# spencerkent/vision-transform-codes

Measured on AMD Instinct MI355X. Metric: patches/sec through 200-iter FISTA + dict update, 1024-atom dict, higher is better.
Workload: dtype f16x3

## Files before the change

### vision-transform-codes_amd/analysis_transforms/fully_connected/ista_fista.py

```python
import ctypes

import torch

import vtc_hip


def run(images, dictionary, sparsity_weight, num_iters, variant='fista',
        initial_codes=None, early_stopping_epsilon=None,
        nonnegative_only=False, hard_threshold=False, precision=None,
        stepsize=None):
  assert variant in ['ista', 'fista']
  lib = vtc_hip.load_library()
  images = vtc_hip.require_device_tensor(images, 'images').contiguous()
  dictionary = vtc_hip.require_device_tensor(
      dictionary, 'dictionary').contiguous()
  b, n = images.shape
  s = dictionary.shape[0]
  assert dictionary.shape[1] == n
  vtc_hip.prepare_device(images.device)
  if initial_codes is not None:
    initial_codes = vtc_hip.require_device_tensor(
        initial_codes, 'initial_codes').contiguous()
    assert tuple(initial_codes.shape) == (b, s)
  images = vtc_hip.aligned16(images)
  dictionary = vtc_hip.aligned16(dictionary)
  initial_codes = vtc_hip.aligned16(initial_codes)
  if num_iters < 1:
    raise UnboundLocalError(
        "local variable 'codes' referenced before assignment")

  mode = vtc_hip.threshold_mode(nonnegative_only, hard_threshold)
  prec = _resolve_precision(precision, b, n, s, early_stopping_epsilon)
  lam = float(sparsity_weight)
  eps = -1.0 if early_stopping_epsilon is None else float(
      early_stopping_epsilon)
  ws_bytes = lib.vtc_fc_ista_fista_workspace_bytes(b, n, s, prec)
  ws = vtc_hip.workspace(ws_bytes, images.device)
  codes = torch.empty((b, s), dtype=torch.float32, device=images.device)
  iters_run = ctypes.c_int(0)
  common = (int(num_iters), vtc_hip.variant_code(variant), mode, eps, prec,
            vtc_hip.ptr(ws), ws.numel(), ctypes.byref(iters_run),
            vtc_hip.current_stream(images.device))
  if (stepsize is None and early_stopping_epsilon is None and
      vtc_hip.device_stepsize_available(n)):
    eta_dev = vtc_hip.stepsize_on_device(
        vtc_hip.gram(dictionary, transpose_a=True), dictionary)
    with vtc_hip.timed_call(images.device):
      status = lib.vtc_fc_ista_fista_dev(
          vtc_hip.ptr(images), vtc_hip.ptr(dictionary),
          vtc_hip.ptr(initial_codes), vtc_hip.ptr(codes), b, n, s,
          vtc_hip.ptr(eta_dev), lam, *common)
    vtc_hip.check(status, 'vtc_fc_ista_fista_dev')
  else:
    if stepsize is None:
      stepsize = vtc_hip.stepsize_from_gram(
          vtc_hip.gram(dictionary, transpose_a=True), dictionary)
    with vtc_hip.timed_call(images.device):
      status = lib.vtc_fc_ista_fista(
          vtc_hip.ptr(images), vtc_hip.ptr(dictionary),
          vtc_hip.ptr(initial_codes), vtc_hip.ptr(codes), b, n, s,
          float(stepsize), lam, *common)
    vtc_hip.check(status, 'vtc_fc_ista_fista')
  run.last_iters = iters_run.value
  return codes


def _resolve_precision(precision, b, n, s, early_stopping_epsilon):
  name = precision if precision is not None else (
      vtc_hip.get_default_precision())
  if name == 'auto':
    fused_ok = (early_stopping_epsilon is None and n == 256 and
                s in (256, 512, 1024) and fused_available())
    tiled_ok = (n % 4 == 0 and s % 4 == 0 and b * s * n >= 240000000 and
                fused_available())
    streamed_ok = (early_stopping_epsilon is None and n == 256 and
                   s > 1024 and s % 256 == 0 and fused_available())
    if fused_ok or streamed_ok:
      return vtc_hip.F16X3
    small_ok = (early_stopping_epsilon is None and n == 64 and
                s in (64, 128, 192))
    if small_ok:
      return vtc_hip.F32
    if early_stopping_epsilon is None and (
        (n == 144 and s in (288, 576)) or (n == 64 and s in (256, 512))):
      return vtc_hip.F32
    return vtc_hip.F16X3 if tiled_ok else vtc_hip.F32
  return vtc_hip.PRECISIONS[name]


def fused_available():
  lib = vtc_hip.load_library()
  return lib.vtc_fc_ista_fista_workspace_bytes(32, 256, 1024,
                                               vtc_hip.BF16X3) > 256
```

### vision-transform-codes_amd/csrc/dict_update.hip

```cpp
#include "common.h"
#include "gemm_f32.h"

namespace vtc {

__global__ void slab_reduce_kernel(const float* __restrict__ slabs, int slices,
                                   int64_t count, float* __restrict__ out) {
  const int64_t stride = (int64_t)gridDim.x * blockDim.x;
  for (int64_t i = (int64_t)blockIdx.x * blockDim.x + threadIdx.x; i < count;
       i += stride) {
    float a[8] = {0.f, 0.f, 0.f, 0.f, 0.f, 0.f, 0.f, 0.f};
    int z = 0;
    for (; z + 8 <= slices; z += 8) {
#pragma unroll
      for (int u = 0; u < 8; ++u)
        a[u] = add_rn(a[u], slabs[(int64_t)(z + u) * count + i]);
    }
    for (int u = 0; z < slices; ++z, ++u)
      a[u] = add_rn(a[u], slabs[(int64_t)z * count + i]);
    out[i] = add_rn(add_rn(add_rn(a[0], a[1]), add_rn(a[2], a[3])),
                    add_rn(add_rn(a[4], a[5]), add_rn(a[6], a[7])));
  }
}

__global__ void slab_reduce_minus_kernel(const float* __restrict__ slabs,
                                         int slices, int64_t count,
                                         const float* __restrict__ X,
                                         float* __restrict__ out,
                                         unsigned* max_out) {
  const int64_t stride = (int64_t)gridDim.x * blockDim.x;
  float mx = 0.f;
  for (int64_t i = (int64_t)blockIdx.x * blockDim.x + threadIdx.x; i < count;
       i += stride) {
    float acc = slabs[i];
    for (int z = 1; z < slices; ++z) acc += slabs[(int64_t)z * count + i];
    const float r = sub_rn(acc, X[i]);
    out[i] = r;
    mx = fmaxf(mx, fabsf(r));
  }
  if (max_out) cx_publish_max_wave(mx, max_out);
}

int launch_slab_reduce_minus(const float* slabs, int slices, int64_t count,
                             const float* X, float* out, hipStream_t st,
                             unsigned* max_out) {
  if (count <= 0) return VTC_OK;
  int64_t blocks = ceil_div(count, 256);
  if (blocks > 4096) blocks = 4096;
  hipLaunchKernelGGL(slab_reduce_minus_kernel, dim3((unsigned)blocks),
                     dim3(256), 0, st, slabs, slices, count, X, out, max_out);
  VTC_LAUNCH_CHECK();
  return VTC_OK;
}

int launch_slab_reduce(const float* slabs, int slices, int64_t count,
                       float* out, hipStream_t st) {
  if (count <= 0) return VTC_OK;
  int64_t blocks = ceil_div(count, 256);
  if (blocks > 2048) blocks = 2048;
  hipLaunchKernelGGL(slab_reduce_kernel, dim3((unsigned)blocks), dim3(256), 0,
                     st, slabs, slices, count, out);
  VTC_LAUNCH_CHECK();
  return VTC_OK;
}

static int gradient_slices(int64_t b, int64_t n, int64_t s) {
  const int64_t tiles = ceil_div(s, kGemmBM) * ceil_div(n, kGemmBN);
  int64_t want = ceil_div(1024, tiles);
  const int64_t cap = ceil_div(b, 64);
  if (want > cap) want = cap;
  if (want > 128) want = 128;
  if (want < 1) want = 1;
  return gemm_effective_slices(b, (int)want);
}

__device__ __forceinline__ void fc_apply_row(
    float* __restrict__ D, const float* __restrict__ G,
    const float* __restrict__ hess, const float* __restrict__ P,
    float alignment_penalty, float batch_f, float stepsize, float lowest,
    int normalize, int64_t row, int64_t n, int lane) {
  float* d = D + row * n;
  const float* g = G + row * n;
  const float* p = P ? P + row * n : nullptr;
  const float denom = hess ? add_rn(hess[row], lowest) : 1.f;
  float sumsq = 0.f;
  for (int64_t j = lane; j < n; j += 64) {
    float grad = g[j] / batch_f;
    if (p) grad = add_rn(grad, mul_rn(alignment_penalty, p[j]));
    float step = mul_rn(stepsize, grad);
    if (hess) step = step / denom;
    const float v = sub_rn(d[j], step);
    d[j] = v;
    sumsq = fmaf(v, v, sumsq);
  }
  if (!normalize) return;
  const float norm = sqrtf(wave_sum(sumsq));
  for (int64_t j = lane; j < n; j += 64) d[j] = d[j] / norm;
}

__global__ __launch_bounds__(256) void fc_apply_kernel(
    float* __restrict__ D, const float* __restrict__ G,
    const float* __restrict__ hess, const float* __restrict__ P,
    float alignment_penalty, float batch_f, float stepsize, float lowest,
    int normalize, int64_t s, int64_t n, int rows_per_block) {
  const int lane = threadIdx.x & 63;
  const int64_t first = (int64_t)blockIdx.x * rows_per_block;
  const int64_t last = first + rows_per_block < s ? first + rows_per_block : s;
  for (int64_t row = first + (threadIdx.x >> 6); row < last; row += 4)
    fc_apply_row(D, G, hess, P, alignment_penalty, batch_f, stepsize, lowest,
                 normalize, row, n, lane);
}
constexpr int kMaxGroup = 256;
constexpr size_t kMaxAlignmentLds = 160 * 1024;

__global__ __launch_bounds__(256) void alignment_slot_kernel(
    const float* __restrict__ D, const int32_t* __restrict__ index,
    const uint8_t* __restrict__ valid, float* __restrict__ slot_grad,
    int64_t n, int m, int normalized) {
  extern __shared__ __attribute__((aligned(16))) float lds[];
  float* rows = lds;
  float* cosines = lds + (size_t)m * n;
  float* norms = cosines + m * m;
  const int g = blockIdx.x;
  const int32_t* idx = index + (int64_t)g * m;
  const uint8_t* ok = valid + (int64_t)g * m;
  int members = 0;
  for (int j = 0; j < m; ++j) members += ok[j] ? 1 : 0;
  for (int64_t e = threadIdx.x; e < (int64_t)members * n; e += blockDim.x) {
    const int r = (int)(e / n);
    const int64_t c = e % n;
    rows[e] = D[(int64_t)idx[r] * n + c];
  }
  __syncthreads();
  const int lane = threadIdx.x & 63, wave = threadIdx.x >> 6;
  for (int pair = wave; pair < members * members; pair += 4) {
    const int i = pair / members, j = pair % members;
    float acc = 0.f;
    for (int64_t c = lane; c < n; c += 64)
      acc = fmaf(rows[(int64_t)i * n + c], rows[(int64_t)j * n + c], acc);
    acc = wave_sum(acc);
    if (lane == 0) cosines[i * m + j] = acc;
  }
  __syncthreads();
  if (!normalized) {
    if (threadIdx.x < members)
      norms[threadIdx.x] = sqrtf(cosines[threadIdx.x * m + threadIdx.x]);
    __syncthreads();
  }
  for (int64_t e = threadIdx.x; e < (int64_t)members * n; e += blockDim.x) {
    const int i = (int)(e / n);
    const int64_t c = e % n;
    const float di = rows[(int64_t)i * n + c];
    float acc = 0.f;
    for (int j = 0; j < members; ++j) {
      const float dj = rows[(int64_t)j * n + c];
      float cs, toward_other, toward_self;
      if (normalized) {
        cs = cosines[i * m + j];
        toward_other = dj;
        toward_self = mul_rn(cs, di);
      } else {
        const float outer = mul_rn(norms[i], norms[j]);
        cs = cosines[i * m + j] / outer;
        toward_other = dj / outer;
        toward_self = mul_rn(cs / mul_rn(norms[i], norms[i]), di);
      }
      acc = add_rn(acc, mul_rn(sign_of(cs), sub_rn(toward_other, toward_self)));
    }
    slot_grad[((int64_t)g * m + i) * n + c] = acc;
  }
}

__global__ void rows_by_atom_sum_kernel(const float* __restrict__ slot_rows,
                                        const int32_t* __restrict__ atom_ptr,
                                        const int32_t* __restrict__ atom_slots,
                                        float* __restrict__ out, int64_t s,
                                        int64_t n) {
  const int64_t a = blockIdx.x;
  if (a >= s) return;
  const int beg = atom_ptr[a], end = atom_ptr[a + 1];
  for (int64_t c = threadIdx.x; c < n; c += blockDim.x) {
    float acc = 0.f;
    for (int t = beg; t < end; ++t)
      acc = add_rn(acc, slot_rows[(int64_t)atom_slots[t] * n + c]);
    out[a * n + c] = acc;
  }
}

__global__ __launch_bounds__(256) void energy_rows_kernel(
    const float* __restrict__ codes, int64_t b, int64_t s, int rows_per_chunk,
    float* __restrict__ partial) {
  const int64_t chunk = blockIdx.y;
  const int64_t j = (int64_t)blockIdx.x * blockDim.x + threadIdx.x;
  if (j >= s) return;
  const int64_t r0 = chunk * rows_per_chunk;
  int64_t r1 = r0 + rows_per_chunk;
  if (r1 > b) r1 = b;
  float acc = 0.f;
  for (int64_t r = r0; r < r1; ++r) {
    const float v = codes[r * s + j];
    acc = fmaf(v, v, acc);
  }
  partial[chunk * s + j] = acc;
}

__global__ __launch_bounds__(256) void energy_maps_kernel(
    const float* __restrict__ codes, int64_t s, int64_t positions,
    float* __restrict__ partial) {
  __shared__ float red[4];
  const int64_t map = blockIdx.x;
  const float* p = codes + map * positions;
  float acc = 0.f;
  for (int64_t i = threadIdx.x; i < positions; i += blockDim.x) {
    const float v = p[i];
    acc = fmaf(v, v, acc);
  }
  acc = wave_sum(acc);
  if ((threadIdx.x & 63) == 0) red[threadIdx.x >> 6] = acc;
  __syncthreads();
  if (threadIdx.x == 0) partial[map] = (red[0] + red[1]) + (red[2] + red[3]);
}

__global__ void hessian_ema_kernel(float* __restrict__ h,
                                   const float* __restrict__ energy,
                                   float batch_f, int64_t s) {
  const int64_t j = (int64_t)blockIdx.x * blockDim.x + threadIdx.x;
  if (j >= s) return;
  const float mean = energy[j] / batch_f;
  h[j] = add_rn(mul_rn(h[j], 0.99f), mean / 100.f);
}

static int energy_chunk_rows(int64_t b) {
  int64_t rows = ceil_div(b, 512);
  if (rows < 32) rows = 32;
  return (int)rows;
}


struct FcGradLayout {
  float* E;
  float* slabs;
  FcGradLayout(Carver& ws, int64_t b, int64_t n, int64_t s) {
    E = ws.take<float>((size_t)b * n);
    slabs = ws.take<float>((size_t)gradient_slices(b, n, s) * s * n);
  }
};

struct SlotGradLayout {
  float* slot_grad;
  SlotGradLayout(Carver& ws, int64_t slots, int64_t n) {
    slot_grad = ws.take<float>((size_t)(slots > 0 ? slots : 1) * n);
  }
};

struct EnergyLayout {
  int64_t chunks;
  float* partial;
  EnergyLayout(Carver& ws, int64_t b, int64_t s, int64_t positions) {
    chunks = positions > 1 ? b : ceil_div(b, energy_chunk_rows(b));
    partial = ws.take<float>((size_t)chunks * s);
  }
};

struct IcaMomentLayout {
  float* S;
  float* slabs;
  IcaMomentLayout(Carver& ws, int64_t b, int64_t s) {
    S = ws.take<float>((size_t)b * s);
    slabs = ws.take<float>((size_t)gradient_slices(b, s, s) * s * s);
  }
};

struct IcaApplyLayout {
  float* T;
  float* U;
  IcaApplyLayout(Carver& ws, int64_t s, int64_t n) {
    T = ws.take<float>((size_t)s * s);
    U = ws.take<float>((size_t)s * n);
  }
};

}

using namespace vtc;

extern "C" int vtc_gram(const float* a, int64_t rows, int64_t cols,
                        int transpose_a, float* gram, void* stream) {
  VTC_REQUIRE(a && gram, "vtc_gram: null pointer");
  VTC_REQUIRE(rows > 0 && cols > 0, "vtc_gram: bad sizes");
  hipStream_t st = as_stream(stream);
  if (transpose_a) {
    EpiStore e{gram, cols};
    return launch_gemm_f32<false, false>(a, cols, a, cols, cols, cols, rows, 1,
                                         e, st);
  }
  EpiStore e{gram, rows};
  return launch_gemm_f32<true, true>(a, cols, a, cols, rows, rows, cols, 1, e,
                                     st);
}

extern "C" size_t vtc_fc_dict_gradient_workspace_bytes(int64_t b, int64_t n,
                                                       int64_t s) {
  if (b <= 0 || n <= 0 || s <= 0) return 256;
  return measured_bytes<FcGradLayout>(b, n, s);
}

extern "C" int vtc_fc_dict_gradient(const float* images,
                                    const float* dictionary,
                                    const float* codes, float* grad_sum,
                                    int64_t b, int64_t n, int64_t s,
                                    void* workspace, size_t workspace_bytes,
                                    void* stream) {
  VTC_REQUIRE(images && dictionary && codes && grad_sum,
              "vtc_fc_dict_gradient: null pointer");
  VTC_REQUIRE(b > 0 && n > 0 && s > 0, "vtc_fc_dict_gradient: bad sizes");
  if (!workspace ||
      workspace_bytes < vtc_fc_dict_gradient_workspace_bytes(b, n, s)) {
    set_error("vtc_fc_dict_gradient: workspace too small");
    return VTC_ERR_WORKSPACE;
  }
  hipStream_t st = as_stream(stream);
  Carver ws(workspace);
  const FcGradLayout L(ws, b, n, s);
  const int slices = gradient_slices(b, n, s);
  EpiMinus e1{L.E, images, n, n};
  int rc = launch_gemm_f32<true, false>(codes, s, dictionary, n, b, n, s, 1,
                                        e1, st);
  if (rc != VTC_OK) return rc;
  if (b <= 512 && gemm_prefers_small(s, n)) {
    EpiStore direct{grad_sum, n};
    return launch_gemm_f32<false, false>(codes, s, L.E, n, s, n, b, 1, direct,
                                         st);
  }
  EpiSlab e2{L.slabs, s * n, n};
  rc = launch_gemm_f32<false, false>(codes, s, L.E, n, s, n, b, slices, e2, st);
  if (rc != VTC_OK) return rc;
  return launch_slab_reduce(L.slabs, slices, s * n, grad_sum, st);
}

__global__ void sign_kernel(const float* __restrict__ x, float* __restrict__ y,
                            int64_t count) {
  const int64_t stride = (int64_t)gridDim.x * blockDim.x;
  for (int64_t i = (int64_t)blockIdx.x * blockDim.x + threadIdx.x; i < count;
       i += stride)
    y[i] = sign_of(x[i]);
}

__global__ void ica_center_kernel(const float* __restrict__ moment_sum,
                                  float* __restrict__ T, float batch_f,
                                  int64_t s) {
  const int64_t total = s * s;
  const int64_t stride = (int64_t)gridDim.x * blockDim.x;
  for (int64_t i = (int64_t)blockIdx.x * blockDim.x + threadIdx.x; i < total;
       i += stride) {
    const float eye = (i / s == i % s) ? 1.f : 0.f;
    T[i] = sub_rn(moment_sum[i] / batch_f, eye);
  }
}

__global__ void axpy_rn_kernel(float* __restrict__ D,
                               const float* __restrict__ U, float stepsize,
                               int64_t count) {
  const int64_t stride = (int64_t)gridDim.x * blockDim.x;
  for (int64_t i = (int64_t)blockIdx.x * blockDim.x + threadIdx.x; i < count;
       i += stride)
    D[i] = add_rn(D[i], mul_rn(stepsize, U[i]));
}

static unsigned stream_grid(int64_t total) {
  int64_t blocks = ceil_div(total, 256);
  if (blocks > 4096) blocks = 4096;
  if (blocks < 1) blocks = 1;
  return (unsigned)blocks;
}

extern "C" int vtc_fc_residual(const float* images, const float* dictionary,
                               const float* codes, float* residual, int64_t b,
                               int64_t n, int64_t s, void* stream) {
  VTC_REQUIRE((images && dictionary && codes && residual) || b == 0,
              "vtc_fc_residual: null pointer");
  VTC_REQUIRE(b >= 0 && n > 0 && s > 0, "vtc_fc_residual: bad sizes");
  if (b == 0) return VTC_OK;
  EpiMinus e{residual, images, n, n};
  return launch_gemm_f32<true, false>(codes, s, dictionary, n, b, n, s, 1, e,
                                      as_stream(stream));
}

extern "C" size_t vtc_subspace_alignment_gradient_workspace_bytes(
    int64_t slots, int64_t n) {
  return measured_bytes<SlotGradLayout>(slots, n);
}

extern "C" int vtc_subspace_alignment_gradient(
    const float* dictionary, const int32_t* index, const uint8_t* valid,
    const int32_t* atom_ptr, const int32_t* atom_slots, float* penalty_grad,
    int64_t s, int64_t n, int64_t groups, int64_t m, int dict_is_normalized,
    void* workspace, size_t workspace_bytes, void* stream) {
  VTC_REQUIRE(dictionary && index && valid && atom_ptr && atom_slots &&
                  penalty_grad, "vtc_subspace_alignment_gradient: null");
  VTC_REQUIRE(s > 0 && n > 0 && groups > 0 && m > 0,
              "vtc_subspace_alignment_gradient: bad sizes");
  const size_t lds_bytes = ((size_t)m * n + (size_t)m * m + m) * sizeof(float);
  if (m > kMaxGroup || lds_bytes > kMaxAlignmentLds) {
    set_error("vtc_subspace_alignment_gradient: group of %lld atoms x %lld "
              "pixels exceeds the LDS tile", (long long)m, (long long)n);
    return VTC_ERR_UNSUPPORTED;
  }
  if (!workspace || workspace_bytes <
      vtc_subspace_alignment_gradient_workspace_bytes(groups * m, n)) {
    set_error("vtc_subspace_alignment_gradient: workspace too small");
    return VTC_ERR_WORKSPACE;
  }
  hipStream_t st = as_stream(stream);
  Carver ws(workspace);
  float* slot_grad = SlotGradLayout(ws, groups * m, n).slot_grad;
  VTC_HIP_CHECK(hipMemsetAsync(slot_grad, 0,
                               (size_t)groups * m * n * sizeof(float), st));
  if (lds_bytes > 64 * 1024)
    VTC_HIP_CHECK(hipFuncSetAttribute(
        reinterpret_cast<const void*>(alignment_slot_kernel),
        hipFuncAttributeMaxDynamicSharedMemorySize, (int)lds_bytes));
  hipLaunchKernelGGL(alignment_slot_kernel, dim3((unsigned)groups), dim3(256),
                     lds_bytes, st, dictionary, index, valid, slot_grad, n,
                     (int)m, dict_is_normalized);
  VTC_LAUNCH_CHECK();
  hipLaunchKernelGGL(rows_by_atom_sum_kernel, dim3((unsigned)s), dim3(256), 0,
                     st, slot_grad, atom_ptr, atom_slots, penalty_grad, s, n);
  VTC_LAUNCH_CHECK();
  return VTC_OK;
}

extern "C" int vtc_fc_dict_apply(float* dictionary, const float* grad_sum,
                                 const float* hessian_diagonal,
                                 const float* penalty_grad,
                                 float alignment_penalty, int64_t global_batch,
                                 float stepsize, float lowest_code_val,
                                 int normalize, int64_t s, int64_t n,
                                 void* stream) {
  VTC_REQUIRE(dictionary && grad_sum, "vtc_fc_dict_apply: null pointer");
  VTC_REQUIRE(s > 0 && n > 0 && global_batch > 0,
              "vtc_fc_dict_apply: bad sizes");
  int64_t rows = 32;
  while (rows > 4 && ((rows / 2) * n * 4) % 128 == 0) rows /= 2;
  if (reinterpret_cast<uintptr_t>(dictionary) % 128 != 0) rows = s;
  hipLaunchKernelGGL(fc_apply_kernel, dim3((unsigned)ceil_div(s, rows)),
                     dim3(256), 0, as_stream(stream), dictionary, grad_sum,
                     hessian_diagonal, penalty_grad, alignment_penalty,
                     (float)global_batch, stepsize, lowest_code_val, normalize,
                     s, n, (int)rows);
  VTC_LAUNCH_CHECK();
  return VTC_OK;
}

extern "C" size_t vtc_code_energy_workspace_bytes(int64_t b, int64_t s,
                                                  int64_t positions) {
  if (b <= 0 || s <= 0) return 256;
  return measured_bytes<EnergyLayout>(b, s, positions);
}

extern "C" int vtc_code_energy(const float* codes, int64_t b, int64_t s,
                               int64_t positions, float* energy,
                               void* workspace, size_t workspace_bytes,
                               void* stream) {
  VTC_REQUIRE(codes && energy, "vtc_code_energy: null pointer");
  VTC_REQUIRE(b > 0 && s > 0 && positions > 0, "vtc_code_energy: bad sizes");
  if (!workspace ||
      workspace_bytes < vtc_code_energy_workspace_bytes(b, s, positions)) {
    set_error("vtc_code_energy: workspace too small");
    return VTC_ERR_WORKSPACE;
  }
  hipStream_t st = as_stream(stream);
  Carver ws(workspace);
  const EnergyLayout L(ws, b, s, positions);
  const int64_t chunks = L.chunks;
  if (positions == 1) {
    const int rows = energy_chunk_rows(b);
    hipLaunchKernelGGL(energy_rows_kernel,
                       dim3((unsigned)ceil_div(s, 256), (unsigned)chunks),
                       dim3(256), 0, st, codes, b, s, rows, L.partial);
  } else {
    hipLaunchKernelGGL(energy_maps_kernel, dim3((unsigned)(b * s)), dim3(256),
                       0, st, codes, s, positions, L.partial);
  }
  VTC_LAUNCH_CHECK();
  return launch_slab_reduce(L.partial, (int)chunks, s, energy, st);
}

extern "C" int vtc_hessian_ema(float* hessian_diagonal, const float* energy,
                               int64_t global_batch, int64_t s, void* stream) {
  VTC_REQUIRE(hessian_diagonal && energy, "vtc_hessian_ema: null pointer");
  VTC_REQUIRE(s > 0 && global_batch > 0, "vtc_hessian_ema: bad sizes");
  hipLaunchKernelGGL(hessian_ema_kernel, dim3((unsigned)ceil_div(s, 256)),
                     dim3(256), 0, as_stream(stream), hessian_diagonal, energy,
                     (float)global_batch, s);
  VTC_LAUNCH_CHECK();
  return VTC_OK;
}

extern "C" size_t vtc_ica_moment_workspace_bytes(int64_t b, int64_t s) {
  if (b <= 0 || s <= 0) return 256;
  return measured_bytes<IcaMomentLayout>(b, s);
}

extern "C" int vtc_ica_moment(const float* codes, float* moment_sum, int64_t b,
                              int64_t s, void* workspace,
                              size_t workspace_bytes, void* stream) {
  VTC_REQUIRE(codes && moment_sum, "vtc_ica_moment: null pointer");
  VTC_REQUIRE(b > 0 && s > 0, "vtc_ica_moment: bad sizes");
  if (!workspace || workspace_bytes < vtc_ica_moment_workspace_bytes(b, s)) {
    set_error("vtc_ica_moment: workspace too small");
    return VTC_ERR_WORKSPACE;
  }
  hipStream_t st = as_stream(stream);
  Carver ws(workspace);
  const IcaMomentLayout L(ws, b, s);
  const int slices = gradient_slices(b, s, s);
  hipLaunchKernelGGL(sign_kernel, dim3(stream_grid(b * s)), dim3(256), 0, st,
                     codes, L.S, b * s);
  VTC_LAUNCH_CHECK();
  EpiSlab e{L.slabs, s * s, s};
  int rc = launch_gemm_f32<false, false>(codes, s, L.S, s, s, s, b, slices, e,
                                         st);
  if (rc != VTC_OK) return rc;
  return launch_slab_reduce(L.slabs, slices, s * s, moment_sum, st);
}

extern "C" size_t vtc_ica_apply_workspace_bytes(int64_t s, int64_t n) {
  if (s <= 0 || n <= 0) return 256;
  return measured_bytes<IcaApplyLayout>(s, n);
}

extern "C" int vtc_ica_apply(float* dictionary, const float* moment_sum,
                             int64_t global_batch, int64_t s, int64_t n,
                             float stepsize, void* workspace,
                             size_t workspace_bytes, void* stream) {
  VTC_REQUIRE(dictionary && moment_sum, "vtc_ica_apply: null pointer");
  VTC_REQUIRE(global_batch > 0 && s > 0 && n > 0, "vtc_ica_apply: bad sizes");
  if (!workspace || workspace_bytes < vtc_ica_apply_workspace_bytes(s, n)) {
    set_error("vtc_ica_apply: workspace too small");
    return VTC_ERR_WORKSPACE;
  }
  hipStream_t st = as_stream(stream);
  Carver ws(workspace);
  const IcaApplyLayout L(ws, s, n);
  hipLaunchKernelGGL(ica_center_kernel, dim3(stream_grid(s * s)), dim3(256), 0,
                     st, moment_sum, L.T, (float)global_batch, s);
  VTC_LAUNCH_CHECK();
  EpiStore e{L.U, n};
  int rc = launch_gemm_f32<true, false>(L.T, s, dictionary, n, s, n, s, 1, e,
                                        st);
  if (rc != VTC_OK) return rc;
  hipLaunchKernelGGL(axpy_rn_kernel, dim3(stream_grid(s * n)), dim3(256), 0,
                     st, dictionary, L.U, stepsize, s * n);
  VTC_LAUNCH_CHECK();
  return VTC_OK;
}
```

### vision-transform-codes_amd/csrc/fc_fused.h

```cpp
#pragma once
#include "common.h"
#include <vector>

namespace vtc {

bool fused_shape_supported(int64_t b, int64_t n, int64_t s, int precision);
size_t fused_workspace_bytes(int64_t b, int64_t n, int64_t s, int precision);
int run_fused(const float* images, const float* dictionary,
              const float* initial_codes, float* codes, int64_t b, int64_t n,
              int64_t s, float eta, const float* eta_dev,
              float sparsity_weight, int num_iters, int variant,
              int threshold, int precision, void* workspace,
              size_t workspace_bytes, int* iters_run, hipStream_t st);
int fused_max_iters();
const float* fista_beta_table_on_this_device();

void fista_betas(int num_iters, std::vector<float>* out);

}
```

### vision-transform-codes_amd/csrc/fc_fused.hip

```cpp
#include "fc_fused.h"
#include "fused_common.h"

#include <stdlib.h>
#include <mutex>
#include <vector>

namespace vtc {

struct FusedParams {
  const float* images;
  const float* init;
  float* codes;
  const uint4* packA[2];
  const uint4* packT[2];
  const float* betas;
  int64_t b;
  int s;
  int num_iters;
  int fista;
  float eta, cutoff;
  const float* eta_dev;
  float lam;
  const float* dscale;
  unsigned long long* stamps;
};

constexpr int kYxRow = 272;
constexpr int kRxRow = 528;
constexpr int kYxPart = 32 * kYxRow;
constexpr int kRxPart = 32 * kRxRow;

template <int NPH, int NP>
struct FusedLds {
  static constexpr int CREG_WANT = (NP == 1) ? 1 : 3;
  static constexpr int CREG = CREG_WANT < NPH ? CREG_WANT : NPH;
  static constexpr int CL = NPH - CREG;
  static constexpr int cst_bytes = CL * 16384;
  static constexpr int yx_bytes = 2 * NP * kYxPart;
  static constexpr int rx_bytes = NP * kRxPart;
  static constexpr int stat_bytes = 2 * 4 * 32 * 4;
  static constexpr int total = cst_bytes + yx_bytes + rx_bytes + stat_bytes;
};

template <int NPH, int NP, int MODE, bool F16 = false, bool STAMP = false>
__global__ __launch_bounds__(256, 1) void fused_fista_kernel(FusedParams P) {
  static_assert(!F16 || NP == 2, "the f16 split exists as three products only");
  using L = FusedLds<NPH, NP>;
  constexpr int CREG = L::CREG;
  constexpr int CR = CREG > 0 ? CREG : 1;
  constexpr int RING = (NP == 1) ? 16 : 8;
  extern __shared__ __attribute__((aligned(16))) char smem[];
  char* Cst = smem;
  char* Yx = smem + L::cst_bytes;
  char* Rx = Yx + L::yx_bytes;
  float* Stat = reinterpret_cast<float*>(Rx + L::rx_bytes);

  const int tid = threadIdx.x;
  const int lane = tid & 63;
  const int w = __builtin_amdgcn_readfirstlane(tid >> 6);
  const int r = lane & 31, h = lane >> 5;
  const int64_t patch = (int64_t)blockIdx.x * kFP + r;
  const bool live = patch < P.b;
  const int s = P.s;

  const unsigned pack_bytes_total = (unsigned)s * kFN * 2u;
  const unsigned a_wave_off = (unsigned)w * (16u * 64u * 16u);
  const unsigned t_wave_off = (unsigned)(2 * w) * (8u * 64u * 16u);
  __amdgpu_buffer_rsrc_t rsA[NP], rsT[NP];
#pragma unroll
  for (int part = 0; part < NP; ++part) {
    rsA[part] = __builtin_amdgcn_make_buffer_rsrc(
        (void*)((const char*)P.packA[part] + a_wave_off), 0,
        (int)(pack_bytes_total - a_wave_off), 0x00020000);
    rsT[part] = __builtin_amdgcn_make_buffer_rsrc(
        (void*)((const char*)P.packT[part] + t_wave_off), 0,
        (int)(pack_bytes_total - t_wave_off), 0x00020000);
  }
  const unsigned frag_voff = (unsigned)lane * 16u;
#define VTC_LOAD_A(part, p, i) \
  buffer_load16(rsA[part], frag_voff, (unsigned)(((4 * (p)) * 16 + (i)) * 1024))
#define VTC_LOAD_T(part, p, nb, ks) \
  buffer_load16(rsT[part], frag_voff,  \
                (unsigned)((((p) * 8 + (nb)) * 8 + (ks)) * 1024))

  const int yx_rd = r * kYxRow + 16 * h;
  const int yx_wr = r * kYxRow + 64 * w + 8 * h;
  const int rx_rd = r * kRxRow + 16 * h;
  const int rx_wr = r * kRxRow + 128 * w + 8 * h;
  const int cst_ln = w * 4096 + lane * 16;

  f32x16 Y[NPH];
  f32x16 Cr[CR];
  f32x16 Xr[2];
  f32x16 Racc[2];
  uint4 ring[NP][RING];

#pragma unroll
  for (int nb = 0; nb < 2; ++nb) {
#pragma unroll
    for (int g = 0; g < 4; ++g) {
      float4 v = make_float4(0.f, 0.f, 0.f, 0.f);
      if (live)
        v = *reinterpret_cast<const float4*>(
            P.images + patch * kFN + 64 * w + 32 * nb + 8 * g + 4 * h);
      Xr[nb][4 * g + 0] = v.x;
      Xr[nb][4 * g + 1] = v.y;
      Xr[nb][4 * g + 2] = v.z;
      Xr[nb][4 * g + 3] = v.w;
    }
  }
  const bool warm = (P.init != nullptr);
#pragma unroll
  for (int p = 0; p < NPH; ++p) {
#pragma unroll
    for (int g = 0; g < 4; ++g) {
      float4 v = make_float4(0.f, 0.f, 0.f, 0.f);
      if (warm && live)
        v = *reinterpret_cast<const float4*>(
            P.init + patch * s + kPhaseAtoms * p + 32 * w + 8 * g + 4 * h);
      Y[p][4 * g + 0] = v.x;
      Y[p][4 * g + 1] = v.y;
      Y[p][4 * g + 2] = v.z;
      Y[p][4 * g + 3] = v.w;
    }
  }
  float sigma_y = 1.f, inv_sigma_y = 1.f;
  float sigma_d = 1.f, inv_sigma_d = 1.f;
  if (F16) {
    float sx = 0.f, sy = 0.f;
#pragma unroll
    for (int nb = 0; nb < 2; ++nb)
#pragma unroll
      for (int e = 0; e < 16; ++e) sx += Xr[nb][e] * Xr[nb][e];
    if (warm) {
#pragma unroll
      for (int p = 0; p < NPH; ++p)
#pragma unroll
        for (int e = 0; e < 16; ++e) sy += Y[p][e] * Y[p][e];
    }
    sx += __shfl_xor(sx, 32, 64);
    sy += __shfl_xor(sy, 32, 64);
    float* red = reinterpret_cast<float*>(Rx);
    if (h == 0) {
      red[w * 64 + r] = sx;
      red[w * 64 + 32 + r] = sy;
    }
    __syncthreads();
    float tx = 0.f, ty = 0.f;
#pragma unroll
    for (int v = 0; v < 4; ++v) {
      tx += red[v * 64 + r];
      ty += red[v * 64 + 32 + r];
    }
    __syncthreads();
    const float m2 = fmaxf(tx, ty);
    int e2 = 0;
    if (m2 > 0.f && m2 < __builtin_inff()) e2 = ilogbf(m2) >> 1;
    e2 = e2 < -60 ? -60 : (e2 > 60 ? 60 : e2);
    sigma_y = ldexpf(1.f, 8 - e2);
    inv_sigma_y = ldexpf(1.f, e2 - 8);
    sigma_d = P.dscale[0];
    inv_sigma_d = P.dscale[1];
    const float sx_scale = sigma_d * sigma_y;
#pragma unroll
    for (int nb = 0; nb < 2; ++nb)
#pragma unroll
      for (int e = 0; e < 16; ++e) Xr[nb][e] *= sx_scale;
#pragma unroll
    for (int p = 0; p < NPH; ++p)
#pragma unroll
      for (int e = 0; e < 16; ++e) Y[p][e] *= sigma_y;
  }
  float eta = P.eta, cutoff_l = P.cutoff;
  if (P.eta_dev) {
    eta = *P.eta_dev;
    cutoff_l = mul_rn(P.lam, eta);
  }
  if (F16) {
    eta = eta * (0.5f * inv_sigma_d);
    cutoff_l = cutoff_l * sigma_y;
  }
  const float r_scale = F16 ? 2.f * inv_sigma_d : 1.f;
  int xr_calls = 0;
#pragma unroll
  for (int p = 0; p < NPH; ++p) {
#pragma unroll
    for (int g = 0; g < 4; ++g) {
      if (p < CREG) {
#pragma unroll
        for (int q = 0; q < 4; ++q)
          Cr[p < CREG ? p : 0][4 * g + q] = Y[p][4 * g + q];
      } else {
        *reinterpret_cast<float4*>(Cst + cst_ln + (p - CREG) * 16384 +
                                   g * 1024) =
            make_float4(Y[p][4 * g + 0], Y[p][4 * g + 1], Y[p][4 * g + 2],
                        Y[p][4 * g + 3]);
      }
    }
  }
#pragma unroll
  for (int nb = 0; nb < 2; ++nb)
#pragma unroll
    for (int e = 0; e < 16; ++e) Racc[nb][e] = 0.f;

  auto publish_y = [&](const f32x16& y, int buf) {
#pragma unroll
    for (int g = 0; g < 4; ++g) {
      const float v4[4] = {y[4 * g], y[4 * g + 1], y[4 * g + 2], y[4 * g + 3]};
      uint2 hi, lo;
      split_packed<F16, 4, NP == 2>(v4, hi, lo);
      char* dst = Yx + buf * NP * kYxPart + yx_wr + 16 * g;
      *reinterpret_cast<uint2*>(dst) = hi;
      if (NP == 2) *reinterpret_cast<uint2*>(dst + kYxPart) = lo;
    }
  };

#define VTC_SEG_IS_T(sg) (((sg) >= 2 && ((sg) % 2) == 0) || (sg) == 2 * NPH - 1)
#define VTC_SEG_PHASE(sg)                                        \
  ((sg) == 0 ? 0                                                 \
             : (sg) == 2 * NPH - 1 ? NPH - 1                     \
                                   : ((sg) % 2 ? ((sg) + 1) / 2 : (sg) / 2 - 1))
#define VTC_LOAD_SEG(part, sg, i)                                          \
  (VTC_SEG_IS_T(sg) ? VTC_LOAD_T(part, VTC_SEG_PHASE(sg), (i) & 1, (i) >> 1) \
                    : VTC_LOAD_A(part, VTC_SEG_PHASE(sg), (i)))
#define VTC_REFILL(sg, i)                                                   \
  {                                                                         \
    const int j_ = (i) + RING;                                              \
    const int sg_ = (j_ < 16) ? (sg) : (((sg) + 1) % (2 * NPH));            \
    const int i_ = (j_ < 16) ? j_ : j_ - 16;                                \
    _Pragma("unroll") for (int part = 0; part < NP; ++part)                 \
        ring[part][(i) % RING] = VTC_LOAD_SEG(part, sg_, i_);               \
  }

  auto step3 = [&](int p, int buf, bool pipe, int sg, auto&& between) {
    uint4 yb_next[NP];
#pragma unroll
    for (int part = 0; part < NP; ++part)
      yb_next[part] = *reinterpret_cast<const uint4*>(
          Yx + (buf * NP + part) * kYxPart + yx_rd);
#pragma unroll
    for (int ks = 0; ks < 8; ++ks) {
      uint4 yb[NP];
#pragma unroll
      for (int part = 0; part < NP; ++part) {
        yb[part] = yb_next[part];
        if (ks + 1 < 8)
          yb_next[part] = *reinterpret_cast<const uint4*>(
              Yx + (buf * NP + part) * kYxPart + yx_rd + 32 * (ks + 1));
      }
#pragma unroll
      for (int nb = 0; nb < 2; ++nb) {
        const int i = 2 * ks + nb;
        uint4 a[NP];
#pragma unroll
        for (int part = 0; part < NP; ++part)
          a[part] = pipe ? ring[part][i % RING] : VTC_LOAD_T(part, p, nb, ks);
        Racc[nb] = mfma16<F16>(a[0], yb[0], Racc[nb]);
        if constexpr (NP == 2) {
          Racc[nb] = mfma16<F16>(a[0], yb[1], Racc[nb]);
          Racc[nb] = mfma16<F16>(a[1], yb[0], Racc[nb]);
        }
        between(i);
        if (pipe) VTC_REFILL(sg, i)
        __builtin_amdgcn_sched_barrier(0);
      }
    }
  };
  auto nothing = [](int) {};

  auto exchange_r = [&]() {
    float v[2][16];
#pragma unroll
    for (int nb = 0; nb < 2; ++nb)
#pragma unroll
      for (int e = 0; e < 16; ++e) {
        v[nb][e] = sub_rn(Racc[nb][e], Xr[nb][e]);
        if (F16) v[nb][e] *= r_scale;
      }
    if (F16) {
      float m = 0.f;
#pragma unroll
      for (int nb = 0; nb < 2; ++nb)
#pragma unroll
        for (int e = 0; e < 16; ++e) m = fmaxf(m, fabsf(v[nb][e]));
      m = fmaxf(m, __shfl_xor(m, 32, 64));
      float f = 1.f;
      if (xr_calls > 0) {
        const float* prev = Stat + ((xr_calls - 1) & 1) * 128;
        const float Mx = fmaxf(fmaxf(prev[r], prev[32 + r]),
                               fmaxf(prev[64 + r], prev[96 + r]));
        if (Mx > 2048.f && Mx < __builtin_inff())
          f = ldexpf(1.f, 9 - ilogbf(Mx));
      }
      if (h == 0) Stat[(xr_calls & 1) * 128 + w * 32 + r] = m * f;
      ++xr_calls;
      if (__any(f != 1.f)) {
#pragma unroll
        for (int p = 0; p < NPH; ++p)
#pragma unroll
          for (int e = 0; e < 16; ++e) Y[p][e] *= f;
#pragma unroll
        for (int p = 0; p < CR; ++p)
#pragma unroll
          for (int e = 0; e < 16; ++e) Cr[p][e] *= f;
#pragma unroll
        for (int pl = 0; pl < L::CL; ++pl)
#pragma unroll
          for (int g = 0; g < 4; ++g) {
            float4* c4 = reinterpret_cast<float4*>(Cst + cst_ln + pl * 16384 +
                                                   g * 1024);
            float4 c = *c4;
            c.x *= f; c.y *= f; c.z *= f; c.w *= f;
            *c4 = c;
          }
#pragma unroll
        for (int nb = 0; nb < 2; ++nb)
#pragma unroll
          for (int e = 0; e < 16; ++e) {
            Xr[nb][e] *= f;
            v[nb][e] *= f;
          }
        cutoff_l *= f;
        inv_sigma_y *= 1.f / f;
      }
    }
#pragma unroll
    for (int nb = 0; nb < 2; ++nb) {
#pragma unroll
      for (int g = 0; g < 4; ++g) {
        const float v4[4] = {v[nb][4 * g], v[nb][4 * g + 1], v[nb][4 * g + 2],
                             v[nb][4 * g + 3]};
        uint2 hi, lo;
        split_packed<F16, 4, NP == 2>(v4, hi, lo);
        char* dst = Rx + rx_wr + 64 * nb + 16 * g;
        *reinterpret_cast<uint2*>(dst) = hi;
        if (NP == 2) *reinterpret_cast<uint2*>(dst + kRxPart) = lo;
      }
    }
#pragma unroll
    for (int nb = 0; nb < 2; ++nb)
#pragma unroll
      for (int e = 0; e < 16; ++e) Racc[nb][e] = 0.f;
    __syncthreads();
  };

  if (warm) {
#pragma unroll
    for (int p = 0; p < NPH; ++p) {
      publish_y(Y[p], p & 1);
      __syncthreads();
      step3(p, p & 1, false, 0, nothing);
    }
  }
  exchange_r();

#pragma unroll
  for (int i = 0; i < RING; ++i)
#pragma unroll
    for (int part = 0; part < NP; ++part)
      ring[part][i] = VTC_LOAD_SEG(part, 0, i);

  const bool fista = P.fista != 0;
  unsigned long long acc_t[5] = {0, 0, 0, 0, 0};
  unsigned long long t0 = 0, t1 = 0;
#define VTC_STAMP(slot)                    \
  if (STAMP) {                             \
    t1 = stamp_now();                      \
    acc_t[slot] += t1 - t0;                \
    t0 = t1;                               \
  }
  if (STAMP) t0 = stamp_now();

  f32x16 Gb[2];
  float4 cold4;
  float cn4[4];

  auto epilogue_elem = [&](int p, int e, const f32x16& Gp, float beta) {
    const int g = e >> 2, k = e & 3;
    if (MODE == 7) {
      const float cn = Y[p][e] + Gp[e];
      Y[p][e] = cn;
      cn4[k] = cn;
      if (k == 3) {
        if (p < CREG) {
#pragma unroll
          for (int q = 0; q < 4; ++q) Cr[p < CREG ? p : 0][4 * g + q] = cn4[q];
        } else {
          *reinterpret_cast<float4*>(Cst + cst_ln + (p - CREG) * 16384 +
                                     g * 1024) =
              make_float4(cn4[0], cn4[1], cn4[2], cn4[3]);
        }
      }
      return;
    }
    if (k == 0) {
      if (p < CREG) {
        cold4 = make_float4(Cr[p < CREG ? p : 0][4 * g + 0],
                            Cr[p < CREG ? p : 0][4 * g + 1],
                            Cr[p < CREG ? p : 0][4 * g + 2],
                            Cr[p < CREG ? p : 0][4 * g + 3]);
      } else {
        cold4 = *reinterpret_cast<const float4*>(
            Cst + cst_ln + (p - CREG) * 16384 + g * 1024);
      }
    }
    const float co = (k == 0) ? cold4.x : (k == 1) ? cold4.y
                   : (k == 2) ? cold4.z : cold4.w;
    const float c = sub_rn(Y[p][e], mul_rn(eta, Gp[e]));
    const float cn = shrink_fast<MODE>(c, cutoff_l);
    Y[p][e] = fista ? add_rn(cn, mul_rn(beta, sub_rn(cn, co))) : cn;
    cn4[k] = cn;
    if (k == 3) {
      if (p < CREG) {
#pragma unroll
        for (int q = 0; q < 4; ++q) Cr[p < CREG ? p : 0][4 * g + q] = cn4[q];
      } else {
        *reinterpret_cast<float4*>(Cst + cst_ln + (p - CREG) * 16384 +
                                   g * 1024) =
            make_float4(cn4[0], cn4[1], cn4[2], cn4[3]);
      }
      const float v4[4] = {Y[p][4 * g], Y[p][4 * g + 1], Y[p][4 * g + 2],
                           Y[p][4 * g + 3]};
      uint2 hi, lo;
      split_packed<F16, 4, NP == 2>(v4, hi, lo);
      char* dst = Yx + (p & 1) * NP * kYxPart + yx_wr + 16 * g;
      *reinterpret_cast<uint2*>(dst) = hi;
      if (NP == 2) *reinterpret_cast<uint2*>(dst + kYxPart) = lo;
    }
  };

  auto step1 = [&](int p, int sg, bool overlap, float beta) {
    f32x16& G = Gb[p & 1];
#pragma unroll
    for (int e = 0; e < 16; ++e) G[e] = 0.f;
    uint4 rb_next[NP];
#pragma unroll
    for (int part = 0; part < NP; ++part)
      rb_next[part] =
          *reinterpret_cast<const uint4*>(Rx + part * kRxPart + rx_rd);
#pragma unroll
    for (int i = 0; i < 16; ++i) {
      uint4 rb[NP];
#pragma unroll
      for (int part = 0; part < NP; ++part) {
        rb[part] = rb_next[part];
        if (i + 1 < 16)
          rb_next[part] = *reinterpret_cast<const uint4*>(
              Rx + part * kRxPart + rx_rd + 32 * (i + 1));
      }
      G = mfma16<F16>(ring[0][i % RING], rb[0], G);
      if constexpr (NP == 2) {
        G = mfma16<F16>(ring[0][i % RING], rb[1], G);
        G = mfma16<F16>(ring[1][i % RING], rb[0], G);
      }
      if (overlap) {
        epilogue_elem(p - 1, i, Gb[(p - 1) & 1], beta);
        __builtin_amdgcn_sched_barrier(0);
      }
      VTC_REFILL(sg, i)
      __builtin_amdgcn_sched_barrier(0);
    }
  };

  for (int it = 0; it < P.num_iters; ++it) {
    const float beta = fista ? P.betas[it] : 0.f;
    step1(0, 0, false, beta);
    VTC_STAMP(0)
#pragma unroll
    for (int p = 0; p < NPH; ++p) {
      if (p + 1 < NPH) {
        step1(p + 1, 2 * p + 1, true, beta);
        VTC_STAMP(0)
      }
      __syncthreads();
      VTC_STAMP(2)
      if (p + 2 == NPH) {
        step3(p, p & 1, true, 2 * p + 2, [&](int i) {
          epilogue_elem(NPH - 1, i, Gb[(NPH - 1) & 1], beta);
          __builtin_amdgcn_sched_barrier(0);
        });
      } else {
        step3(p, p & 1, true, (p + 1 < NPH) ? 2 * p + 2 : 2 * NPH - 1, nothing);
      }
      VTC_STAMP(3)
    }
    exchange_r();
    VTC_STAMP(4)
  }
  if (STAMP && lane == 0) {
#pragma unroll
    for (int k = 0; k < 5; ++k) atomicAdd(P.stamps + k, acc_t[k]);
    atomicAdd(P.stamps + 7, 1ull);
  }
#undef VTC_STAMP

#pragma unroll
  for (int p = 0; p < NPH; ++p) {
#pragma unroll
    for (int g = 0; g < 4; ++g) {
      float4 v;
      if (p < CREG) {
        v = make_float4(Cr[p < CREG ? p : 0][4 * g + 0],
                        Cr[p < CREG ? p : 0][4 * g + 1],
                        Cr[p < CREG ? p : 0][4 * g + 2],
                        Cr[p < CREG ? p : 0][4 * g + 3]);
      } else {
        v = *reinterpret_cast<const float4*>(Cst + cst_ln +
                                             (p - CREG) * 16384 + g * 1024);
      }
      if (F16) {
        v.x *= inv_sigma_y;
        v.y *= inv_sigma_y;
        v.z *= inv_sigma_y;
        v.w *= inv_sigma_y;
      }
      if (live)
        *reinterpret_cast<float4*>(P.codes + patch * s + kPhaseAtoms * p +
                                   32 * w + 8 * g + 4 * h) = v;
    }
  }
#undef VTC_LOAD_A
#undef VTC_LOAD_T
#undef VTC_LOAD_SEG
#undef VTC_REFILL
#undef VTC_SEG_IS_T
#undef VTC_SEG_PHASE
}

template <int NPH, int NP, int MODE, bool F16 = false, bool STAMP = false>
__global__ __launch_bounds__(256, 1) void fused_fista_kernel16(FusedParams P) {
  static_assert(!F16 || NP == 2, "the f16 split exists as three products only");
  using L = FusedLds<NPH, NP>;
  constexpr int CREG = L::CREG;
  constexpr int CR = CREG > 0 ? CREG : 1;
  constexpr int RING = (NP == 1) ? 16 : 8;
  constexpr int NPROD = (NP == 2) ? 3 : 1;
  extern __shared__ __attribute__((aligned(16))) char smem[];
  char* Cst = smem;
  char* Yx = smem + L::cst_bytes;
  char* Rx = Yx + L::yx_bytes;
  float* Stat = reinterpret_cast<float*>(Rx + L::rx_bytes);

  const int tid = threadIdx.x;
  const int lane = tid & 63;
  const int w = __builtin_amdgcn_readfirstlane(tid >> 6);
  const int c = lane & 15, q = lane >> 4;
  int64_t patch[2];
  bool live[2];
#pragma unroll
  for (int n = 0; n < 2; ++n) {
    patch[n] = (int64_t)blockIdx.x * kFP + 16 * n + c;
    live[n] = patch[n] < P.b;
  }
  const int s = P.s;

  const unsigned pack_bytes_total = (unsigned)s * kFN * 2u;
  const unsigned a_wave_off = (unsigned)w * (16u * 64u * 16u);
  const unsigned t_wave_off = (unsigned)(4 * w) * (4u * 64u * 16u);
  __amdgpu_buffer_rsrc_t rsA[NP], rsT[NP];
#pragma unroll
  for (int part = 0; part < NP; ++part) {
    rsA[part] = __builtin_amdgcn_make_buffer_rsrc(
        (void*)((const char*)P.packA[part] + a_wave_off), 0,
        (int)(pack_bytes_total - a_wave_off), 0x00020000);
    rsT[part] = __builtin_amdgcn_make_buffer_rsrc(
        (void*)((const char*)P.packT[part] + t_wave_off), 0,
        (int)(pack_bytes_total - t_wave_off), 0x00020000);
  }
  const unsigned frag_voff = (unsigned)lane * 16u;
#define VTC_LOAD_A(part, p, i) \
  buffer_load16(rsA[part], frag_voff, (unsigned)(((4 * (p)) * 16 + (i)) * 1024))
#define VTC_LOAD_T(part, p, nb, ks) \
  buffer_load16(rsT[part], frag_voff,  \
                (unsigned)((((p) * 16 + (nb)) * 4 + (ks)) * 1024))

  const int swap = ((c >> 2) ^ (c >> 3)) & 1;
  const int rd_chunk = 32 * (q >> 1) + 16 * ((q & 1) ^ swap);
  const int wr_chunk = 16 * ((q >> 1) ^ swap) + 8 * (q & 1);
  const int yx_rd = c * kYxRow + rd_chunk;
  const int yx_wr = c * kYxRow + 64 * w + wr_chunk;
  const int rx_rd = c * kRxRow + rd_chunk;
  const int rx_wr = c * kRxRow + 128 * w + wr_chunk;
  const int cst_ln = w * 4096 + lane * 16;
  constexpr int kYxHalf = 16 * kYxRow, kRxHalf = 16 * kRxRow;

  f32x16 Y[NPH];
  f32x16 Cr[CR];
  f32x4 Xr[4][2];
  f32x4 Racc[4][2];
  uint4 ring[NP][RING];

#pragma unroll
  for (int nb = 0; nb < 4; ++nb) {
#pragma unroll
    for (int n = 0; n < 2; ++n) {
      float4 v = make_float4(0.f, 0.f, 0.f, 0.f);
      if (live[n])
        v = *reinterpret_cast<const float4*>(P.images + patch[n] * kFN + 64 * w +
                                             16 * nb + 4 * q);
      Xr[nb][n][0] = v.x;
      Xr[nb][n][1] = v.y;
      Xr[nb][n][2] = v.z;
      Xr[nb][n][3] = v.w;
    }
  }
  const bool warm = (P.init != nullptr);
#pragma unroll
  for (int p = 0; p < NPH; ++p) {
#pragma unroll
    for (int g = 0; g < 4; ++g) {
      float4 v = make_float4(0.f, 0.f, 0.f, 0.f);
      if (warm && live[g & 1])
        v = *reinterpret_cast<const float4*>(P.init + patch[g & 1] * s +
                                             kPhaseAtoms * p + 32 * w +
                                             16 * (g >> 1) + 4 * q);
      Y[p][4 * g + 0] = v.x;
      Y[p][4 * g + 1] = v.y;
      Y[p][4 * g + 2] = v.z;
      Y[p][4 * g + 3] = v.w;
    }
  }
  float sigma_y[2] = {1.f, 1.f}, inv_sigma_y[2] = {1.f, 1.f};
  float sigma_d = 1.f, inv_sigma_d = 1.f;
  if (F16) {
    float sx[2] = {0.f, 0.f}, sy[2] = {0.f, 0.f};
#pragma unroll
    for (int nb = 0; nb < 4; ++nb)
#pragma unroll
      for (int n = 0; n < 2; ++n)
#pragma unroll
        for (int k = 0; k < 4; ++k) sx[n] += Xr[nb][n][k] * Xr[nb][n][k];
    if (warm) {
#pragma unroll
      for (int p = 0; p < NPH; ++p)
#pragma unroll
        for (int e = 0; e < 16; ++e) sy[(e >> 2) & 1] += Y[p][e] * Y[p][e];
    }
    float* red = reinterpret_cast<float*>(Rx);
#pragma unroll
    for (int n = 0; n < 2; ++n) {
      sx[n] += __shfl_xor(sx[n], 16, 64);
      sx[n] += __shfl_xor(sx[n], 32, 64);
      sy[n] += __shfl_xor(sy[n], 16, 64);
      sy[n] += __shfl_xor(sy[n], 32, 64);
      if (q == 0) {
        red[w * 64 + 16 * n + c] = sx[n];
        red[w * 64 + 32 + 16 * n + c] = sy[n];
      }
    }
    __syncthreads();
    float m2[2];
#pragma unroll
    for (int n = 0; n < 2; ++n) {
      float tx = 0.f, ty = 0.f;
#pragma unroll
      for (int v = 0; v < 4; ++v) {
        tx += red[v * 64 + 16 * n + c];
        ty += red[v * 64 + 32 + 16 * n + c];
      }
      m2[n] = fmaxf(tx, ty);
    }
    __syncthreads();
    sigma_d = P.dscale[0];
    inv_sigma_d = P.dscale[1];
#pragma unroll
    for (int n = 0; n < 2; ++n) {
      int e2 = 0;
      if (m2[n] > 0.f && m2[n] < __builtin_inff()) e2 = ilogbf(m2[n]) >> 1;
      e2 = e2 < -60 ? -60 : (e2 > 60 ? 60 : e2);
      sigma_y[n] = ldexpf(1.f, 8 - e2);
      inv_sigma_y[n] = ldexpf(1.f, e2 - 8);
      const float sx_scale = sigma_d * sigma_y[n];
#pragma unroll
      for (int nb = 0; nb < 4; ++nb)
#pragma unroll
        for (int k = 0; k < 4; ++k) Xr[nb][n][k] *= sx_scale;
    }
#pragma unroll
    for (int p = 0; p < NPH; ++p)
#pragma unroll
      for (int e = 0; e < 16; ++e) Y[p][e] *= sigma_y[(e >> 2) & 1];
  }
  float eta = P.eta, cutoff = P.cutoff;
  if (P.eta_dev) {
    eta = *P.eta_dev;
    cutoff = mul_rn(P.lam, eta);
  }
  float cutoff_l[2] = {cutoff, cutoff};
  if (F16) {
    eta = eta * (0.5f * inv_sigma_d);
    cutoff_l[0] = cutoff * sigma_y[0];
    cutoff_l[1] = cutoff * sigma_y[1];
  }
  const float r_scale = F16 ? 2.f * inv_sigma_d : 1.f;
  int xr_calls = 0;
#pragma unroll
  for (int p = 0; p < NPH; ++p) {
#pragma unroll
    for (int g = 0; g < 4; ++g) {
      if (p < CREG) {
#pragma unroll
        for (int k = 0; k < 4; ++k)
          Cr[p < CREG ? p : 0][4 * g + k] = Y[p][4 * g + k];
      } else {
        *reinterpret_cast<float4*>(Cst + cst_ln + (p - CREG) * 16384 +
                                   g * 1024) =
            make_float4(Y[p][4 * g + 0], Y[p][4 * g + 1], Y[p][4 * g + 2],
                        Y[p][4 * g + 3]);
      }
    }
  }
#pragma unroll
  for (int nb = 0; nb < 4; ++nb)
#pragma unroll
    for (int n = 0; n < 2; ++n)
#pragma unroll
      for (int k = 0; k < 4; ++k) Racc[nb][n][k] = 0.f;

  auto publish_group = [&](const f32x16& y, int g, int buf) {
    const float v4[4] = {y[4 * g], y[4 * g + 1], y[4 * g + 2], y[4 * g + 3]};
    uint2 hi, lo;
    split_packed<F16, 4, NP == 2>(v4, hi, lo);
    char* dst = Yx + buf * NP * kYxPart + yx_wr + 32 * (g >> 1) +
                kYxHalf * (g & 1);
    *reinterpret_cast<uint2*>(dst) = hi;
    if (NP == 2) *reinterpret_cast<uint2*>(dst + kYxPart) = lo;
  };

#define VTC_SEG_IS_T(sg) (((sg) >= 2 && ((sg) % 2) == 0) || (sg) == 2 * NPH - 1)
#define VTC_SEG_PHASE(sg)                                        \
  ((sg) == 0 ? 0                                                 \
             : (sg) == 2 * NPH - 1 ? NPH - 1                     \
                                   : ((sg) % 2 ? ((sg) + 1) / 2 : (sg) / 2 - 1))
#define VTC_LOAD_SEG(part, sg, i)                                          \
  (VTC_SEG_IS_T(sg) ? VTC_LOAD_T(part, VTC_SEG_PHASE(sg), (i) & 3, (i) >> 2) \
                    : VTC_LOAD_A(part, VTC_SEG_PHASE(sg), (i)))
#define VTC_REFILL(sg, i)                                                   \
  {                                                                         \
    const int j_ = (i) + RING;                                              \
    const int sg_ = (j_ < 16) ? (sg) : (((sg) + 1) % (2 * NPH));            \
    const int i_ = (j_ < 16) ? j_ : j_ - 16;                                \
    _Pragma("unroll") for (int part = 0; part < NP; ++part)                 \
        ring[part][(i) % RING] = VTC_LOAD_SEG(part, sg_, i_);               \
  }
#define VTC_MFMA_PAIR(acc0, acc1, a, b)                                     \
  _Pragma("unroll") for (int prod = 0; prod < NPROD; ++prod) {              \
    acc0 = mfma_k32<F16>(a[prod == 2], b[0][prod == 1], acc0);              \
    acc1 = mfma_k32<F16>(a[prod == 2], b[1][prod == 1], acc1);              \
  }

  auto step3 = [&](int p, int buf, bool pipe, int sg, auto&& between) {
    uint4 yb[2][NP], yb_next[2][NP];
#pragma unroll
    for (int n = 0; n < 2; ++n)
#pragma unroll
      for (int part = 0; part < NP; ++part)
        yb_next[n][part] = *reinterpret_cast<const uint4*>(
            Yx + (buf * NP + part) * kYxPart + yx_rd + kYxHalf * n);
#pragma unroll
    for (int i = 0; i < 16; ++i) {
      const int ks = i >> 2, nb = i & 3;
      if (nb == 0) {
#pragma unroll
        for (int n = 0; n < 2; ++n)
#pragma unroll
          for (int part = 0; part < NP; ++part) yb[n][part] = yb_next[n][part];
      }
      if (nb < 2 && ks + 1 < 4) {
#pragma unroll
        for (int part = 0; part < NP; ++part)
          yb_next[nb][part] = *reinterpret_cast<const uint4*>(
              Yx + (buf * NP + part) * kYxPart + yx_rd + kYxHalf * nb +
              64 * (ks + 1));
      }
      uint4 a[NP];
#pragma unroll
      for (int part = 0; part < NP; ++part)
        a[part] = pipe ? ring[part][i % RING] : VTC_LOAD_T(part, p, nb, ks);
      VTC_MFMA_PAIR(Racc[nb][0], Racc[nb][1], a, yb)
      between(i);
      if (pipe) VTC_REFILL(sg, i)
      __builtin_amdgcn_sched_barrier(0);
    }
  };
  auto nothing = [](int) {};

  auto exchange_r = [&]() {
    float v[4][2][4];
#pragma unroll
    for (int nb = 0; nb < 4; ++nb)
#pragma unroll
      for (int n = 0; n < 2; ++n)
#pragma unroll
        for (int k = 0; k < 4; ++k) {
          v[nb][n][k] = sub_rn(Racc[nb][n][k], Xr[nb][n][k]);
          if (F16) v[nb][n][k] *= r_scale;
        }
    if (F16) {
      float f[2] = {1.f, 1.f};
#pragma unroll
      for (int n = 0; n < 2; ++n) {
        float m = 0.f;
#pragma unroll
        for (int nb = 0; nb < 4; ++nb)
#pragma unroll
          for (int k = 0; k < 4; ++k) m = fmaxf(m, fabsf(v[nb][n][k]));
        m = fmaxf(m, __shfl_xor(m, 16, 64));
        m = fmaxf(m, __shfl_xor(m, 32, 64));
        const int row = 16 * n + c;
        if (xr_calls > 0) {
          const float* prev = Stat + ((xr_calls - 1) & 1) * 128;
          const float Mx = fmaxf(fmaxf(prev[row], prev[32 + row]),
                                 fmaxf(prev[64 + row], prev[96 + row]));
          if (Mx > 2048.f && Mx < __builtin_inff())
            f[n] = ldexpf(1.f, 9 - ilogbf(Mx));
        }
        if (q == 0) Stat[(xr_calls & 1) * 128 + w * 32 + row] = m * f[n];
      }
      ++xr_calls;
      if (__any(f[0] != 1.f || f[1] != 1.f)) {
#pragma unroll
        for (int p = 0; p < NPH; ++p)
#pragma unroll
          for (int e = 0; e < 16; ++e) Y[p][e] *= f[(e >> 2) & 1];
#pragma unroll
        for (int p = 0; p < CR; ++p)
#pragma unroll
          for (int e = 0; e < 16; ++e) Cr[p][e] *= f[(e >> 2) & 1];
#pragma unroll
        for (int pl = 0; pl < L::CL; ++pl)
#pragma unroll
          for (int g = 0; g < 4; ++g) {
            float4* c4 = reinterpret_cast<float4*>(Cst + cst_ln + pl * 16384 +
                                                   g * 1024);
            float4 cc = *c4;
            const float fg = f[g & 1];
            cc.x *= fg; cc.y *= fg; cc.z *= fg; cc.w *= fg;
            *c4 = cc;
          }
#pragma unroll
        for (int n = 0; n < 2; ++n) {
#pragma unroll
          for (int nb = 0; nb < 4; ++nb)
#pragma unroll
            for (int k = 0; k < 4; ++k) {
              Xr[nb][n][k] *= f[n];
              v[nb][n][k] *= f[n];
            }
          cutoff_l[n] *= f[n];
          inv_sigma_y[n] *= 1.f / f[n];
        }
      }
    }
#pragma unroll
    for (int nb = 0; nb < 4; ++nb) {
#pragma unroll
      for (int n = 0; n < 2; ++n) {
        const float v4[4] = {v[nb][n][0], v[nb][n][1], v[nb][n][2], v[nb][n][3]};
        uint2 hi, lo;
        split_packed<F16, 4, NP == 2>(v4, hi, lo);
        char* dst = Rx + rx_wr + 32 * nb + kRxHalf * n;
        *reinterpret_cast<uint2*>(dst) = hi;
        if (NP == 2) *reinterpret_cast<uint2*>(dst + kRxPart) = lo;
      }
    }
#pragma unroll
    for (int nb = 0; nb < 4; ++nb)
#pragma unroll
      for (int n = 0; n < 2; ++n)
#pragma unroll
        for (int k = 0; k < 4; ++k) Racc[nb][n][k] = 0.f;
    __syncthreads();
  };

  if (warm) {
#pragma unroll
    for (int p = 0; p < NPH; ++p) {
#pragma unroll
      for (int g = 0; g < 4; ++g) publish_group(Y[p], g, p & 1);
      __syncthreads();
      step3(p, p & 1, false, 0, nothing);
    }
  }
  exchange_r();

#pragma unroll
  for (int i = 0; i < RING; ++i)
#pragma unroll
    for (int part = 0; part < NP; ++part)
      ring[part][i] = VTC_LOAD_SEG(part, 0, i);

  const bool fista = P.fista != 0;
  unsigned long long acc_t[5] = {0, 0, 0, 0, 0};
  unsigned long long t0 = 0, t1 = 0;
#define VTC_STAMP(slot)                    \
  if (STAMP) {                             \
    t1 = stamp_now();                      \
    acc_t[slot] += t1 - t0;                \
    t0 = t1;                               \
  }
  if (STAMP) t0 = stamp_now();

  f32x4 Gb[2][4];
  float4 cold4;
  float cn4[4];

  auto epilogue_elem = [&](int p, int e, const f32x4 (&Gp)[4], float beta) {
    const int g = e >> 2, k = e & 3;
    if (MODE == 7) {
      const float cn = Y[p][e] + Gp[g][k];
      Y[p][e] = cn;
      cn4[k] = cn;
      if (k == 3) {
        if (p < CREG) {
#pragma unroll
          for (int j = 0; j < 4; ++j) Cr[p < CREG ? p : 0][4 * g + j] = cn4[j];
        } else {
          *reinterpret_cast<float4*>(Cst + cst_ln + (p - CREG) * 16384 +
                                     g * 1024) =
              make_float4(cn4[0], cn4[1], cn4[2], cn4[3]);
        }
      }
      return;
    }
    if (k == 0) {
      if (p < CREG) {
        cold4 = make_float4(Cr[p < CREG ? p : 0][4 * g + 0],
                            Cr[p < CREG ? p : 0][4 * g + 1],
                            Cr[p < CREG ? p : 0][4 * g + 2],
                            Cr[p < CREG ? p : 0][4 * g + 3]);
      } else {
        cold4 = *reinterpret_cast<const float4*>(
            Cst + cst_ln + (p - CREG) * 16384 + g * 1024);
      }
    }
    const float co = (k == 0) ? cold4.x : (k == 1) ? cold4.y
                   : (k == 2) ? cold4.z : cold4.w;
    const float cv = sub_rn(Y[p][e], mul_rn(eta, Gp[g][k]));
    const float cn = shrink_fast<MODE>(cv, cutoff_l[g & 1]);
    Y[p][e] = fista ? add_rn(cn, mul_rn(beta, sub_rn(cn, co))) : cn;
    cn4[k] = cn;
    if (k == 3) {
      if (p < CREG) {
#pragma unroll
        for (int j = 0; j < 4; ++j) Cr[p < CREG ? p : 0][4 * g + j] = cn4[j];
      } else {
        *reinterpret_cast<float4*>(Cst + cst_ln + (p - CREG) * 16384 +
                                   g * 1024) =
            make_float4(cn4[0], cn4[1], cn4[2], cn4[3]);
      }
      publish_group(Y[p], g, p & 1);
    }
  };

  auto step1 = [&](int p, int sg, bool overlap, float beta) {
    f32x4 (&G)[4] = Gb[p & 1];
#pragma unroll
    for (int g = 0; g < 4; ++g)
#pragma unroll
      for (int k = 0; k < 4; ++k) G[g][k] = 0.f;
    uint4 rb[2][NP], rb_next[2][NP];
#pragma unroll
    for (int n = 0; n < 2; ++n)
#pragma unroll
      for (int part = 0; part < NP; ++part)
        rb_next[n][part] = *reinterpret_cast<const uint4*>(
            Rx + part * kRxPart + rx_rd + kRxHalf * n);
#pragma unroll
    for (int i = 0; i < 16; ++i) {
      const int ks = i >> 1, m = i & 1;
      if (m == 0) {
#pragma unroll
        for (int n = 0; n < 2; ++n)
#pragma unroll
          for (int part = 0; part < NP; ++part) rb[n][part] = rb_next[n][part];
      }
      if (ks + 1 < 8) {
#pragma unroll
        for (int part = 0; part < NP; ++part)
          rb_next[m][part] = *reinterpret_cast<const uint4*>(
              Rx + part * kRxPart + rx_rd + kRxHalf * m + 64 * (ks + 1));
      }
      uint4 a[NP];
#pragma unroll
      for (int part = 0; part < NP; ++part) a[part] = ring[part][i % RING];
      VTC_MFMA_PAIR(G[2 * m], G[2 * m + 1], a, rb)
      if (overlap) {
        epilogue_elem(p - 1, i, Gb[(p - 1) & 1], beta);
        __builtin_amdgcn_sched_barrier(0);
      }
      VTC_REFILL(sg, i)
      __builtin_amdgcn_sched_barrier(0);
    }
  };

  for (int it = 0; it < P.num_iters; ++it) {
    const float beta = fista ? P.betas[it] : 0.f;
    step1(0, 0, false, beta);
    VTC_STAMP(0)
#pragma unroll
    for (int p = 0; p < NPH; ++p) {
      if (p + 1 < NPH) {
        step1(p + 1, 2 * p + 1, true, beta);
        VTC_STAMP(0)
      }
      __syncthreads();
      VTC_STAMP(2)
      if (p + 2 == NPH) {
        step3(p, p & 1, true, 2 * p + 2, [&](int i) {
          epilogue_elem(NPH - 1, i, Gb[(NPH - 1) & 1], beta);
          __builtin_amdgcn_sched_barrier(0);
        });
      } else {
        step3(p, p & 1, true, (p + 1 < NPH) ? 2 * p + 2 : 2 * NPH - 1, nothing);
      }
      VTC_STAMP(3)
    }
    exchange_r();
    VTC_STAMP(4)
  }
  if (STAMP && lane == 0) {
#pragma unroll
    for (int k = 0; k < 5; ++k) atomicAdd(P.stamps + k, acc_t[k]);
    atomicAdd(P.stamps + 7, 1ull);
  }
#undef VTC_STAMP

#pragma unroll
  for (int p = 0; p < NPH; ++p) {
#pragma unroll
    for (int g = 0; g < 4; ++g) {
      float4 v;
      if (p < CREG) {
        v = make_float4(Cr[p < CREG ? p : 0][4 * g + 0],
                        Cr[p < CREG ? p : 0][4 * g + 1],
                        Cr[p < CREG ? p : 0][4 * g + 2],
                        Cr[p < CREG ? p : 0][4 * g + 3]);
      } else {
        v = *reinterpret_cast<const float4*>(Cst + cst_ln +
                                             (p - CREG) * 16384 + g * 1024);
      }
      if (F16) {
        v.x *= inv_sigma_y[g & 1];
        v.y *= inv_sigma_y[g & 1];
        v.z *= inv_sigma_y[g & 1];
        v.w *= inv_sigma_y[g & 1];
      }
      if (live[g & 1])
        *reinterpret_cast<float4*>(P.codes + patch[g & 1] * s + kPhaseAtoms * p +
                                   32 * w + 16 * (g >> 1) + 4 * q) = v;
    }
  }
#undef VTC_LOAD_A
#undef VTC_LOAD_T
#undef VTC_LOAD_SEG
#undef VTC_REFILL
#undef VTC_MFMA_PAIR
#undef VTC_SEG_IS_T
#undef VTC_SEG_PHASE
}

}

namespace vtc {

static int phases_for(int64_t s) { return (int)(s / kPhaseAtoms); }

bool fused_shape_supported(int64_t b, int64_t n, int64_t s, int precision) {
  if (n != kFN || b <= 0) return false;
  if (s % kPhaseAtoms != 0) return false;
  const int nph = phases_for(s);
  if (!(nph == 2 || nph == 4 || nph == 8)) return false;
  return precision == VTC_BF16 || precision == VTC_BF16X3 ||
         precision == VTC_F16X3;
}

static int fused_parts(int precision) { return precision == VTC_BF16 ? 1 : 2; }

struct FusedLayout {
  unsigned short* packs[4] = {nullptr, nullptr, nullptr, nullptr};
  float* dscale;
  FusedLayout(Carver& ws, int64_t s, int parts) {
    for (int part = 0; part < parts; ++part) {
      packs[2 * part] = ws.take<unsigned short>((size_t)s * kFN);
      packs[2 * part + 1] = ws.take<unsigned short>((size_t)s * kFN);
    }
    dscale = ws.take<float>(2);
  }
};

size_t fused_workspace_bytes(int64_t b, int64_t n, int64_t s, int precision) {
  if (!fused_shape_supported(b, n, s, precision)) return 256;
  return measured_bytes<FusedLayout>(s, fused_parts(precision));
}

static bool default_tile16(int precision) {
  return precision == VTC_F16X3 || precision == VTC_BF16;
}
static bool use_tile16(int precision) {
  const char* v = getenv("VTC_FUSED_TILE");
  if (v && v[0] == '1' && v[1] == '6' && v[2] == 0) return true;
  if (v && v[0] == '3' && v[1] == '2' && v[2] == 0) return false;
  return default_tile16(precision);
}

template <int NPH, int NP, int MODE, bool F16, bool STAMP, bool TILE16>
static auto fused_kernel() {
  if constexpr (TILE16)
    return fused_fista_kernel16<NPH, NP, MODE, F16, STAMP>;
  else
    return fused_fista_kernel<NPH, NP, MODE, F16, STAMP>;
}

template <int NPH, int NP, int MODE, bool F16, bool TILE16>
static int launch_fused(const FusedParams& P, hipStream_t st) {
  using L = FusedLds<NPH, NP>;
  auto kernel = fused_kernel<NPH, NP, MODE, F16, false, TILE16>();
  static unsigned long long configured = 0;
  if (first_use_on_this_device(&configured)) {
    VTC_HIP_CHECK(hipFuncSetAttribute(
        reinterpret_cast<const void*>(kernel),
        hipFuncAttributeMaxDynamicSharedMemorySize, L::total));
  }
  const unsigned grid = (unsigned)ceil_div(P.b, kFP);
  hipLaunchKernelGGL(kernel, dim3(grid), dim3(256), L::total, st, P);
  VTC_LAUNCH_CHECK();
  return VTC_OK;
}

template <int NPH, int NP, bool F16, bool TILE16>
static int launch_stamped(FusedParams P, hipStream_t st) {
  using L = FusedLds<NPH, NP>;
  static const bool no_epilogue = getenv("VTC_FUSED_NOEPI") != nullptr;
  auto kernel = no_epilogue
                    ? fused_kernel<NPH, NP, 7, F16, true, TILE16>()
                    : fused_kernel<NPH, NP, VTC_SOFT, F16, true, TILE16>();
  unsigned long long* dev = nullptr;
  VTC_HIP_CHECK(hipMalloc(&dev, 8 * sizeof(unsigned long long)));
  VTC_HIP_CHECK(hipMemsetAsync(dev, 0, 8 * sizeof(unsigned long long), st));
  VTC_HIP_CHECK(hipFuncSetAttribute(
      reinterpret_cast<const void*>(kernel),
      hipFuncAttributeMaxDynamicSharedMemorySize, L::total));
  P.stamps = dev;
  hipLaunchKernelGGL(kernel, dim3((unsigned)ceil_div(P.b, kFP)), dim3(256),
                     L::total, st, P);
  VTC_LAUNCH_CHECK();
  unsigned long long host[8];
  VTC_HIP_CHECK(hipMemcpyAsync(host, dev, sizeof(host), hipMemcpyDeviceToHost,
                               st));
  VTC_HIP_CHECK(hipStreamSynchronize(st));
  VTC_HIP_CHECK(hipFree(dev));
  const char* names[5] = {"step1+epi", "epi-alone", "barrier", "step3",
                          "exchange"};
  double total = 0;
  for (int k = 0; k < 5; ++k) total += (double)host[k];
  const double per = (double)host[7] * P.num_iters * NPH;
  for (int k = 0; k < 5; ++k)
    fprintf(stderr, "[vtc stamps] %-9s %5.1f%%  %8.0f cycles/phase/wave\n",
            names[k], 100.0 * host[k] / total, host[k] / per);
  return VTC_OK;
}

template <int NPH, int NP, bool F16, bool TILE16>
static int dispatch_mode(const FusedParams& P, int threshold, hipStream_t st) {
  static const bool stamps = getenv("VTC_FUSED_STAMPS") != nullptr;
  if (stamps && threshold == VTC_SOFT && NPH == 8 && NP == 2)
    return launch_stamped<NPH, NP, F16, TILE16>(P, st);
  switch (threshold) {
    case VTC_SOFT: return launch_fused<NPH, NP, VTC_SOFT, F16, TILE16>(P, st);
    case VTC_SOFT_NONNEG:
      return launch_fused<NPH, NP, VTC_SOFT_NONNEG, F16, TILE16>(P, st);
    case VTC_HARD: return launch_fused<NPH, NP, VTC_HARD, F16, TILE16>(P, st);
    default: return launch_fused<NPH, NP, VTC_HARD_NONNEG, F16, TILE16>(P, st);
  }
}

template <int NP, bool F16, bool TILE16>
static int dispatch_phases(const FusedParams& P, int threshold,
                           hipStream_t st) {
  switch (phases_for(P.s)) {
    case 2: return dispatch_mode<2, NP, F16, TILE16>(P, threshold, st);
    case 4: return dispatch_mode<4, NP, F16, TILE16>(P, threshold, st);
    case 8: return dispatch_mode<8, NP, F16, TILE16>(P, threshold, st);
  }
  set_error("fused FISTA: unsupported atom count %d", P.s);
  return VTC_ERR_UNSUPPORTED;
}

constexpr int kBetaTable = 16384;
const float* fista_beta_table_on_this_device() {
  static float* tables[64] = {nullptr};
  static std::mutex guard;
  int dev = 0;
  if (hipGetDevice(&dev) != hipSuccess || dev < 0 || dev > 63) return nullptr;
  std::lock_guard<std::mutex> lock(guard);
  if (tables[dev]) return tables[dev];
  std::vector<float> host;
  fista_betas(kBetaTable, &host);
  float* table = nullptr;
  if (hipMalloc(&table, sizeof(float) * kBetaTable) != hipSuccess)
    return nullptr;
  if (hipMemcpy(table, host.data(), sizeof(float) * kBetaTable,
                hipMemcpyHostToDevice) != hipSuccess) {
    (void)hipFree(table);
    return nullptr;
  }
  tables[dev] = table;
  return table;
}

int fused_max_iters() { return kBetaTable; }

int run_fused(const float* images, const float* dictionary,
              const float* initial_codes, float* codes, int64_t b, int64_t n,
              int64_t s, float eta, const float* eta_dev,
              float sparsity_weight, int num_iters, int variant,
              int threshold, int precision, void* workspace,
              size_t workspace_bytes, int* iters_run, hipStream_t st) {
  if (!fused_shape_supported(b, n, s, precision)) {
    set_error("fused FISTA: unsupported shape");
    return VTC_ERR_UNSUPPORTED;
  }
  if (num_iters > kBetaTable) {
    set_error("fused FISTA: at most %d iterations per call", kBetaTable);
    return VTC_ERR_UNSUPPORTED;
  }
  if (!workspace ||
      workspace_bytes < fused_workspace_bytes(b, n, s, precision)) {
    set_error("fused FISTA: workspace too small");
    return VTC_ERR_WORKSPACE;
  }
  const float* betas_dev = fista_beta_table_on_this_device();
  if (!betas_dev) {
    set_error("fused FISTA: could not place the momentum table on the device");
    return VTC_ERR_HIP;
  }
  const int parts = fused_parts(precision);
  const bool f16 = (precision == VTC_F16X3);
  Carver ws(workspace);
  FusedParams P;
  const FusedLayout L(ws, s, parts);
  unsigned short* const* packs = L.packs;
  float* dscale = L.dscale;
  if (f16) {
    hipLaunchKernelGGL(dictionary_scale_kernel, dim3(1), dim3(1024), 0, st,
                       dictionary, (int64_t)s * kFN, dscale);
    VTC_LAUNCH_CHECK();
  }
  const bool tile16 = use_tile16(precision);
  auto pack = f16 ? (tile16 ? pack_dictionary_kernel<true, true>
                            : pack_dictionary_kernel<true, false>)
                  : (tile16 ? pack_dictionary_kernel<false, true>
                            : pack_dictionary_kernel<false, false>);
  hipLaunchKernelGGL(pack, dim3(256), dim3(256), 0, st, dictionary, (int)s,
                     packs[0], packs[1], packs[2], packs[3], dscale);
  VTC_LAUNCH_CHECK();
  P.images = images;
  P.init = initial_codes;
  P.codes = codes;
  for (int part = 0; part < 2; ++part) {
    P.packA[part] = reinterpret_cast<const uint4*>(packs[2 * (part % parts)]);
    P.packT[part] =
        reinterpret_cast<const uint4*>(packs[2 * (part % parts) + 1]);
  }
  P.betas = betas_dev;
  P.b = b;
  P.s = (int)s;
  P.num_iters = num_iters;
  P.fista = (variant == VTC_FISTA) ? 1 : 0;
  P.eta = eta;
  P.eta_dev = eta_dev;
  P.lam = sparsity_weight;
  P.cutoff = sparsity_weight * eta;
  P.dscale = dscale;
  P.stamps = nullptr;
  int rc;
  if (tile16)
    rc = f16          ? dispatch_phases<2, true, true>(P, threshold, st)
         : parts == 2 ? dispatch_phases<2, false, true>(P, threshold, st)
                      : dispatch_phases<1, false, true>(P, threshold, st);
  else
    rc = f16          ? dispatch_phases<2, true, false>(P, threshold, st)
         : parts == 2 ? dispatch_phases<2, false, false>(P, threshold, st)
                      : dispatch_phases<1, false, false>(P, threshold, st);
  if (rc == VTC_OK && iters_run) *iters_run = num_iters;
  return rc;
}

}

extern "C" int vtc_init(void) {
  if (!vtc::fista_beta_table_on_this_device()) {
    vtc::set_error("vtc_init: could not place the momentum table on the device");
    return VTC_ERR_HIP;
  }
  return VTC_OK;
}
```

### vision-transform-codes_amd/csrc/fc_inference.hip

```cpp
#include "common.h"
#include "gemm_f32.h"
#include "gemm_x3.h"
#include "epi_prox.h"
#include "fc_fused.h"
#include "fused_stream.h"
#include "fc_small.h"

#include <math.h>
#include <vector>

namespace vtc {

struct EpiProx {
  float* Y;
  float* C;
  int64_t ld;
  float eta, cutoff, beta;
  int mode;
  int fista;
  double* delta_sum;
  double local;
  const float* eta_dev = nullptr;
  float lam = 0.f;
  float* Yo = nullptr;
  float* Co = nullptr;
  __device__ __forceinline__ void resolve() {
    if (eta_dev) {
      eta = *eta_dev;
      cutoff = mul_rn(lam, eta);
    }
  }

  static constexpr bool kElemFetch = true;
  struct Fetched {
    float y, c;
  };
  __device__ __forceinline__ Fetched fetch(int64_t row, int64_t col) const {
    const int64_t i = row * ld + col;
    Fetched f;
    f.y = Y[i];
    f.c = fista ? C[i] : 0.f;
    return f;
  }
  __device__ __forceinline__ void apply(int64_t row, int64_t col, float g, int,
                                        const Fetched& f) {
    const int64_t i = row * ld + col;
    const float c = shrink(sub_rn(f.y, mul_rn(eta, g)), cutoff, mode);
    float d;
    if (fista) {
      d = sub_rn(c, f.c);
      Yo[i] = add_rn(c, mul_rn(beta, d));
    } else {
      d = sub_rn(c, f.y);
    }
    Co[i] = c;
    if (delta_sum) local += (double)(fabsf(d) / eta);
  }
  __device__ __forceinline__ void block_end() {
    if (!delta_sum) return;
    const double w = wave_sum(local);
    if ((threadIdx.x & 63) == 0) atomicAdd(delta_sum, w);
  }
};

void fista_betas(int num_iters, std::vector<float>* out) {
  out->resize(num_iters);
  double t = 1.0;
  for (int k = 0; k < num_iters; ++k) {
    const double t_next = (1.0 + sqrt(1.0 + 4.0 * t * t)) / 2.0;
    (*out)[k] = (float)((t - 1.0) / t_next);
    t = t_next;
  }
}

int launch_transpose(const float* in, float* out, int64_t rows, int64_t cols,
                     hipStream_t st);

static size_t generic_workspace_bytes(int64_t b, int64_t n, int64_t s) {
  return measured_bytes<TiledIstaLayout>(b, n, s);
}

static int run_generic(const float* images, const float* dictionary,
                       const float* initial_codes, float* codes, int64_t b,
                       int64_t n, int64_t s, float eta, const float* eta_dev,
                       float lam, int num_iters, int variant, int threshold,
                       float eps, bool x3, bool f16, void* workspace,
                       size_t workspace_bytes, int* iters_run, hipStream_t st) {
  const float cutoff = lam * eta;
  if (workspace_bytes < generic_workspace_bytes(b, n, s) || !workspace) {
    set_error("vtc_fc_ista_fista: workspace too small (%zu < %zu)",
              workspace_bytes, generic_workspace_bytes(b, n, s));
    return VTC_ERR_WORKSPACE;
  }
  Carver ws(workspace);
  const TiledIstaLayout L(ws, b, n, s);
  float* R = L.R;
  float* Dt = L.Dt;
  if (x3 && (n % 4 != 0 || s % 4 != 0)) {
    set_error("vtc_fc_ista_fista: bf16x3 outside the fused kernel needs n "
              "and s to be multiples of 4");
    return VTC_ERR_UNSUPPORTED;
  }
  if (x3 && ((reinterpret_cast<uintptr_t>(dictionary) |
              reinterpret_cast<uintptr_t>(codes)) & 15) != 0)
    x3 = false;
  const int k1_slices = x3 ? gemm_x3_want_slices(b, n, s) : 1;
  double* delta_sum = L.delta_sum;
  unsigned* state = L.state;
  f16 = f16 && x3;
  float* dscale = f16 ? reinterpret_cast<float*>(state) : nullptr;
  unsigned* y_slot[2] = {state + 64, state + 64 + kCxMaxSlotWords};
  unsigned* r_slot[2] = {state + 64 + 2 * kCxMaxSlotWords,
                         state + 64 + 3 * kCxMaxSlotWords};
  if (f16) {
    VTC_HIP_CHECK(hipMemsetAsync(state, 0, kX3StateWords * sizeof(unsigned),
                                 st));
    hipLaunchKernelGGL(cx_array_scale_kernel, dim3(1), dim3(1024), 0, st,
                       dictionary, s * n, dscale);
    VTC_LAUNCH_CHECK();
    if (initial_codes) {
      hipLaunchKernelGGL(cx_array_max_kernel, dim3(1024), dim3(256), 0, st,
                         initial_codes, b * s, y_slot[0]);
      VTC_LAUNCH_CHECK();
    }
  }

  const bool fista = (variant == VTC_FISTA);
  float* Y = fista ? L.Y : codes;
  if (x3) {
    if (!gemm_x3_usable(Y, s, Dt, s) || !gemm_x3_usable(R, n, dictionary, n)) {
      set_error("vtc_fc_ista_fista: split tiles on an unaligned operand");
      return VTC_ERR_INVALID_ARGUMENT;
    }
    int rc = launch_transpose(dictionary, Dt, s, n, st);
    if (rc != VTC_OK) return rc;
  }
  const size_t code_bytes = (size_t)b * s * sizeof(float);
  if (initial_codes) {
    VTC_HIP_CHECK(hipMemcpyAsync(codes, initial_codes, code_bytes,
                                 hipMemcpyDeviceToDevice, st));
    if (fista)
      VTC_HIP_CHECK(hipMemcpyAsync(Y, initial_codes, code_bytes,
                                   hipMemcpyDeviceToDevice, st));
  } else {
    VTC_HIP_CHECK(hipMemsetAsync(codes, 0, code_bytes, st));
    if (fista) VTC_HIP_CHECK(hipMemsetAsync(Y, 0, code_bytes, st));
  }

  std::vector<float> betas;
  fista_betas(num_iters, &betas);
  int done = 0;
  float* Cin = codes;
  float* Cout = L.Cout;
  float* Yout = L.Yout;
  for (int k = 0; k < num_iters; ++k) {
    if (!fista) Y = Cin;
    EpiMinus e1{R, images, n, n};
    X3Scale sc1, sc2;
    if (f16) {
      sc1.b_scale = sc2.b_scale = dscale;
      sc1.a_max = y_slot[k & 1];
      sc1.clear = y_slot[(k + 1) & 1];
      sc2.a_max = r_slot[k & 1];
      sc2.clear = r_slot[(k + 1) & 1];
    }
    int rc;
    if (x3 && k1_slices > 1) {
      EpiSlab es{L.slabs, b * n, n};
      rc = launch_gemm_x3(Y, s, Dt, s, b, n, s, es, st, k1_slices, sc1);
      if (rc == VTC_OK)
        rc = launch_slab_reduce_minus(L.slabs, k1_slices, b * n, images, R, st,
                                      f16 ? r_slot[k & 1] : nullptr);
    } else if (x3 && f16) {
      EpiMinusMax e1m{R, images, n, n, r_slot[k & 1]};
      rc = launch_gemm_x3(Y, s, Dt, s, b, n, s, e1m, st, 1, sc1);
    } else if (x3) {
      rc = launch_gemm_x3(Y, s, Dt, s, b, n, s, e1, st, 1, sc1);
    } else {
      rc = launch_gemm_f32<true, false>(Y, s, dictionary, n, b, n, s, 1, e1,
                                        st);
    }
    if (rc != VTC_OK) return rc;
    if (eps >= 0.f)
      VTC_HIP_CHECK(hipMemsetAsync(delta_sum, 0, sizeof(double), st));
    const bool wide_ok = s % 4 == 0 &&
                         (reinterpret_cast<uintptr_t>(Y) & 15) == 0 &&
                         (reinterpret_cast<uintptr_t>(codes) & 15) == 0;
    if (x3 || (wide_ok && !gemm_prefers_small(b, s))) {
      EpiGroupProx<1, true> e2{Y, Cin, s, eta, cutoff,
                               fista ? betas[k] : 0.f, fista ? 1 : 0,
                               eps >= 0.f ? delta_sum : nullptr, 0.0,
                               threshold, eta_dev, lam};
      e2.Yo = fista ? Yout : Cout;
      e2.Co = Cout;
      if (f16) {
        EpiGroupProx<1, true, true> e2t{Y, Cin, s, eta, cutoff,
                                        fista ? betas[k] : 0.f, fista ? 1 : 0,
                                        eps >= 0.f ? delta_sum : nullptr, 0.0,
                                        threshold, eta_dev, lam};
        e2t.Yo = e2.Yo;
        e2t.Co = e2.Co;
        e2t.track.max_out = y_slot[(k + 1) & 1];
        rc = launch_gemm_x3(R, n, dictionary, n, b, s, n, e2t, st, 1, sc2);
      } else {
        rc = x3 ? launch_gemm_x3(R, n, dictionary, n, b, s, n, e2, st, 1, sc2)
                : launch_gemm_f32<true, true>(R, n, dictionary, n, b, s, n, 1,
                                              e2, st);
      }
    } else {
      EpiProx e2{Y, Cin, s, eta, cutoff, fista ? betas[k] : 0.f, threshold,
                 fista ? 1 : 0, eps >= 0.f ? delta_sum : nullptr, 0.0,
                 eta_dev, lam};
      e2.Yo = Yout;
      e2.Co = Cout;
      rc = launch_gemm_f32<true, true>(R, n, dictionary, n, b, s, n, 1, e2,
                                       st);
    }
    if (rc != VTC_OK) return rc;
    {
      float* t = Cin; Cin = Cout; Cout = t;
      if (fista) { t = Y; Y = Yout; Yout = t; }
    }
    done = k + 1;
    if (eps >= 0.f) {
      double total = 0.0;
      VTC_HIP_CHECK(hipMemcpyAsync(&total, delta_sum, sizeof(double),
                                   hipMemcpyDeviceToHost, st));
      VTC_HIP_CHECK(hipStreamSynchronize(st));
      const float mean = (float)(total / ((double)b * (double)s));
      if (mean < eps && k > 0) break;
    }
  }
  if (Cin != codes)
    VTC_HIP_CHECK(hipMemcpyAsync(codes, Cin, code_bytes,
                                 hipMemcpyDeviceToDevice, st));
  if (iters_run) *iters_run = done;
  return VTC_OK;
}

}

using namespace vtc;

extern "C" size_t vtc_fc_ista_fista_workspace_bytes(int64_t b, int64_t n,
                                                    int64_t s,
                                                    int precision) {
  if (b <= 0 || n <= 0 || s <= 0) return 256;
  const size_t generic = generic_workspace_bytes(b, n, s);
  if (precision == VTC_F32) return generic;
  const size_t fused = fused_workspace_bytes(b, n, s, precision);
  if (precision == VTC_BF16X3 || precision == VTC_F16X3) {
    const size_t streamed = stream_shape_supported(b, n, s, 1, precision)
                                ? stream_workspace_bytes(b, n, s, precision)
                                : 0;
    const size_t most = fused > generic ? fused : generic;
    return most > streamed ? most : streamed;
  }
  return fused;
}

static int fc_ista_fista_impl(const float* images, const float* dictionary,
                              const float* initial_codes, float* codes,
                              int64_t b, int64_t n, int64_t s, float stepsize,
                              const float* stepsize_dev,
                              float sparsity_weight, int num_iters,
                              int variant, int threshold,
                              float early_stopping_epsilon, int precision,
                              void* workspace, size_t workspace_bytes,
                              int* iters_run, void* stream) {
  VTC_REQUIRE(b >= 0 && n > 0 && s > 0, "vtc_fc_ista_fista: bad sizes");
  VTC_REQUIRE(b == 0 || (images && dictionary && codes),
              "vtc_fc_ista_fista: null pointer");
  VTC_REQUIRE(variant == VTC_ISTA || variant == VTC_FISTA,
              "vtc_fc_ista_fista: variant must be ista or fista");
  VTC_REQUIRE(threshold >= VTC_SOFT && threshold <= VTC_HARD_NONNEG,
              "vtc_fc_ista_fista: unknown threshold mode %d", threshold);
  VTC_REQUIRE(num_iters >= 1,
              "vtc_fc_ista_fista: num_iters must be >= 1 (the reference "
              "leaves `codes` unbound for 0)");
  VTC_REQUIRE(precision >= VTC_F32 && precision <= VTC_F16X3,
              "vtc_fc_ista_fista: unknown precision %d", precision);
  if (iters_run) *iters_run = 0;
  if (b == 0) return VTC_OK;
  hipStream_t st = as_stream(stream);
  const bool fused_ok = early_stopping_epsilon < 0.f &&
                        num_iters <= fused_max_iters() &&
                        fused_shape_supported(b, n, s, precision);
  if (precision == VTC_BF16 && !fused_ok) {
    set_error("vtc_fc_ista_fista: VTC_BF16 exists only as the fused kernel "
              "(n == 256, s in {256, 512, 1024}, no early stopping); use "
              "VTC_F16X3, VTC_BF16X3 or VTC_F32");
    return VTC_ERR_UNSUPPORTED;
  }
  const bool aligned16 =
      ((reinterpret_cast<uintptr_t>(images) |
        reinterpret_cast<uintptr_t>(dictionary) |
        reinterpret_cast<uintptr_t>(codes) |
        reinterpret_cast<uintptr_t>(initial_codes)) & 15) == 0;
  if (precision == VTC_BF16 && !aligned16) {
    set_error("vtc_fc_ista_fista: VTC_BF16 exists only as the fused kernel, "
              "which needs %s 16-byte aligned; use VTC_F16X3, VTC_BF16X3 or "
              "VTC_F32",
              first_unaligned16({{"images", images},
                                 {"dictionary", dictionary},
                                 {"initial_codes", initial_codes},
                                 {"codes", codes}}));
    return VTC_ERR_UNSUPPORTED;
  }
  if (precision == VTC_F32 && early_stopping_epsilon < 0.f && aligned16 &&
      num_iters <= fused_max_iters() && small_shape_supported(n, s))
    return run_small(images, dictionary, initial_codes, codes, b, n, s,
                     stepsize, stepsize_dev, sparsity_weight, num_iters,
                     variant, threshold, iters_run, st);
  if (precision == VTC_F32 && early_stopping_epsilon < 0.f && aligned16 &&
      num_iters <= fused_max_iters() && chip16_shape_supported(n, s))
    return run_chip16(images, dictionary, initial_codes, codes, b, n, s,
                      stepsize, stepsize_dev, sparsity_weight, num_iters,
                      variant, threshold, workspace, workspace_bytes,
                      iters_run, st);
  if (precision != VTC_F32 && fused_ok && aligned16)
    return run_fused(images, dictionary, initial_codes, codes, b, n, s,
                     stepsize, stepsize_dev, sparsity_weight, num_iters,
                     variant, threshold, precision, workspace, workspace_bytes,
                     iters_run, st);
  if (precision != VTC_F32 && precision != VTC_BF16 && aligned16 &&
      early_stopping_epsilon < 0.f && num_iters <= fused_max_iters() &&
      stream_shape_supported(b, n, s, 1, precision))
    return run_stream(images, dictionary, initial_codes, codes, b, n, s, 1,
                      stepsize, stepsize_dev, sparsity_weight, num_iters,
                      variant, threshold, precision, workspace,
                      workspace_bytes, iters_run, st);
  return run_generic(images, dictionary, initial_codes, codes, b, n, s,
                     stepsize, stepsize_dev, sparsity_weight, num_iters,
                     variant, threshold, early_stopping_epsilon,
                     precision != VTC_F32, precision == VTC_F16X3, workspace,
                     workspace_bytes, iters_run, st);
}

extern "C" int vtc_fc_ista_fista(const float* images, const float* dictionary,
                                 const float* initial_codes, float* codes,
                                 int64_t b, int64_t n, int64_t s,
                                 float stepsize, float sparsity_weight,
                                 int num_iters, int variant, int threshold,
                                 float early_stopping_epsilon, int precision,
                                 void* workspace, size_t workspace_bytes,
                                 int* iters_run, void* stream) {
  return fc_ista_fista_impl(images, dictionary, initial_codes, codes, b, n, s,
                            stepsize, nullptr, sparsity_weight, num_iters,
                            variant, threshold, early_stopping_epsilon,
                            precision, workspace, workspace_bytes, iters_run,
                            stream);
}

extern "C" int vtc_fc_ista_fista_dev(
    const float* images, const float* dictionary, const float* initial_codes,
    float* codes, int64_t b, int64_t n, int64_t s, const float* stepsize_dev,
    float sparsity_weight, int num_iters, int variant, int threshold,
    float early_stopping_epsilon, int precision, void* workspace,
    size_t workspace_bytes, int* iters_run, void* stream) {
  VTC_REQUIRE(stepsize_dev != nullptr,
              "vtc_fc_ista_fista_dev: stepsize_dev is null");
  return fc_ista_fista_impl(images, dictionary, initial_codes, codes, b, n, s,
                            0.f, stepsize_dev, sparsity_weight, num_iters,
                            variant, threshold, early_stopping_epsilon,
                            precision, workspace, workspace_bytes, iters_run,
                            stream);
}
```

### vision-transform-codes_amd/dict_update_rules/convolutional/_common.py

```python
import ctypes

import torch

import vtc_hip
from vtc_hip import parallel
from utils import convolutions


def descend(images_padded, dictionary, codes, kernel_stride, padding_dims,
            stepsize, num_iters, normalize_dictionary, hessian_diagonal=None,
            lowest_code_val=0.001):
  lib = vtc_hip.load_library()
  images_padded = vtc_hip.require_device_tensor(
      images_padded, 'images_padded').contiguous()
  codes = vtc_hip.require_device_tensor(codes, 'codes').contiguous()
  vtc_hip.require_device_tensor(dictionary, 'dictionary')
  if not dictionary.is_contiguous():
    raise ValueError('dictionary must be contiguous: it is updated in place')
  if hessian_diagonal is not None:
    hessian_diagonal = vtc_hip.require_device_tensor(
        hessian_diagonal, 'hessian_diagonal').contiguous()
  device = images_padded.device
  stream = vtc_hip.current_stream(device)
  geom = convolutions.geometry(images_padded, dictionary, kernel_stride,
                               padding_dims)
  s = geom.s
  kernel_elems = geom.c * geom.kh * geom.kw
  ws = vtc_hip.workspace(
      lib.vtc_conv_dict_gradient_workspace_bytes(ctypes.byref(geom)), device)
  grad_sum = parallel.take(tuple(dictionary.shape), device)
  scratch = torch.empty_like(dictionary)
  total_batch = parallel.global_batch(geom.b, device)
  name = vtc_hip.get_default_precision()
  if name == 'auto':
    name = 'bf16x3' if (geom.s >= 32 and lib.vtc_conv_x3_supported(
        ctypes.byref(geom))) else 'f32'
  elif name != 'f32':
    name = 'bf16x3' if lib.vtc_conv_x3_supported(ctypes.byref(geom)) else (
        'f32')
  for _ in range(num_iters):
    vtc_hip.check(lib.vtc_conv_dict_gradient(
        vtc_hip.ptr(images_padded), vtc_hip.ptr(dictionary),
        vtc_hip.ptr(codes), vtc_hip.ptr(grad_sum), ctypes.byref(geom),
        vtc_hip.PRECISIONS[name], vtc_hip.ptr(ws), ws.numel(), stream),
        'vtc_conv_dict_gradient')
    parallel.all_reduce_sum_(grad_sum)
    vtc_hip.check(lib.vtc_conv_dict_apply(
        vtc_hip.ptr(dictionary), vtc_hip.ptr(grad_sum),
        vtc_hip.ptr(hessian_diagonal), total_batch, float(stepsize),
        float(lowest_code_val), 1 if normalize_dictionary else 0, s,
        kernel_elems, vtc_hip.ptr(scratch), stream), 'vtc_conv_dict_apply')
```

### vision-transform-codes_amd/dict_update_rules/fully_connected/_common.py

```python
import torch

import vtc_hip
from vtc_hip import parallel


def descend(images, dictionary, codes, stepsize, num_iters,
            normalize_dictionary, hessian_diagonal=None, lowest_code_val=0.001,
            penalty=None):
  lib = vtc_hip.load_library()
  images = vtc_hip.require_device_tensor(images, 'images').contiguous()
  codes = vtc_hip.require_device_tensor(codes, 'codes').contiguous()
  vtc_hip.require_device_tensor(dictionary, 'dictionary')
  if not dictionary.is_contiguous():
    raise ValueError('dictionary must be contiguous: it is updated in place')
  b, n = images.shape
  s = dictionary.shape[0]
  assert tuple(codes.shape) == (b, s) and dictionary.shape[1] == n
  if hessian_diagonal is not None:
    hessian_diagonal = vtc_hip.require_device_tensor(
        hessian_diagonal, 'hessian_diagonal').contiguous()
  device = images.device
  stream = vtc_hip.current_stream(device)
  ws = vtc_hip.workspace(lib.vtc_fc_dict_gradient_workspace_bytes(b, n, s),
                         device)
  grad_sum = parallel.take((s, n), device)
  total_batch = parallel.global_batch(b, device)
  for _ in range(num_iters):
    vtc_hip.check(lib.vtc_fc_dict_gradient(
        vtc_hip.ptr(images), vtc_hip.ptr(dictionary), vtc_hip.ptr(codes),
        vtc_hip.ptr(grad_sum), b, n, s, vtc_hip.ptr(ws), ws.numel(), stream),
        'vtc_fc_dict_gradient')
    parallel.all_reduce_sum_(grad_sum)
    pen_weight, pen_grad = 0.0, None
    if penalty is not None:
      pen_weight, pen_fn = penalty
      pen_grad = pen_fn()
    vtc_hip.check(lib.vtc_fc_dict_apply(
        vtc_hip.ptr(dictionary), vtc_hip.ptr(grad_sum),
        vtc_hip.ptr(hessian_diagonal), vtc_hip.ptr(pen_grad),
        float(pen_weight), total_batch, float(stepsize),
        float(lowest_code_val), 1 if normalize_dictionary else 0, s, n,
        stream), 'vtc_fc_dict_apply')
```

### vision-transform-codes_amd/dict_update_rules/fully_connected/ica_natural_gradient.py

```python
import torch

import vtc_hip
from vtc_hip import parallel


def run(dictionary, codes, stepsize=0.001, num_iters=1):
  lib = vtc_hip.load_library()
  dictionary = vtc_hip.require_device_tensor(dictionary, 'dictionary')
  assert dictionary.is_contiguous(), 'dictionary is updated in place'
  codes = vtc_hip.require_device_tensor(codes, 'codes').contiguous()
  b, s = codes.shape
  assert dictionary.shape[0] == s
  n = dictionary.shape[1]
  device = dictionary.device
  stream = vtc_hip.current_stream(device)
  moment = torch.empty((s, s), dtype=torch.float32, device=device)
  ws = vtc_hip.workspace(max(lib.vtc_ica_moment_workspace_bytes(b, s),
                             lib.vtc_ica_apply_workspace_bytes(s, n)), device)
  vtc_hip.check(lib.vtc_ica_moment(
      vtc_hip.ptr(codes), vtc_hip.ptr(moment), b, s, vtc_hip.ptr(ws),
      ws.numel(), stream), 'vtc_ica_moment')
  parallel.all_reduce_sum_(moment)
  total = parallel.global_batch(b, device)
  for _ in range(num_iters):
    vtc_hip.check(lib.vtc_ica_apply(
        vtc_hip.ptr(dictionary), vtc_hip.ptr(moment), total, s, n,
        float(stepsize), vtc_hip.ptr(ws), ws.numel(), stream),
        'vtc_ica_apply')
```

### vision-transform-codes_amd/vtc_hip/__init__.py

```python
import ctypes
import os
import pathlib

import torch

_PKG_ROOT = pathlib.Path(__file__).resolve().parent.parent
LIBRARY_PATH = _PKG_ROOT / 'libvtc_hip.so'

OK, ERR_INVALID_ARGUMENT, ERR_UNSUPPORTED, ERR_WORKSPACE, ERR_HIP = range(5)
ISTA, FISTA = 0, 1
SOFT, SOFT_NONNEG, HARD, HARD_NONNEG = range(4)
F32, BF16X3, BF16, F16X3 = range(4)
PRECISIONS = {'f32': F32, 'bf16x3': BF16X3, 'bf16': BF16, 'f16x3': F16X3}
LOCAL_LUMINANCE, LOCAL_CONTRAST = range(2)
DTYPE_F32, DTYPE_U8 = range(2)
DTYPE_F64 = 2
COLUMN_SUBTRACT, COLUMN_DIVIDE_SQRT = range(2)
ABI_VERSION = 4

_lib = None

_c_f32p = ctypes.c_void_p
_i64 = ctypes.c_int64
_i32 = ctypes.c_int
_f32 = ctypes.c_float
_vp = ctypes.c_void_p
_sz = ctypes.c_size_t


class ConvGeometry(ctypes.Structure):
  _fields_ = [('b', ctypes.c_int64),
              ('c', ctypes.c_int32), ('h', ctypes.c_int32),
              ('w', ctypes.c_int32),
              ('s', ctypes.c_int32), ('kh', ctypes.c_int32),
              ('kw', ctypes.c_int32),
              ('stride_v', ctypes.c_int32), ('stride_h', ctypes.c_int32),
              ('has_padding', ctypes.c_int32),
              ('pad_lead_v', ctypes.c_int32), ('pad_trail_v', ctypes.c_int32),
              ('pad_lead_h', ctypes.c_int32), ('pad_trail_h', ctypes.c_int32)]


_GEOM_P = ctypes.POINTER(ConvGeometry)

SIGNATURES = {
    'vtc_version': (ctypes.c_char_p, []),
    'vtc_last_error': (ctypes.c_char_p, []),
    'vtc_abi_version': (_i32, []),
    'vtc_init': (_i32, []),
    'vtc_gram': (_i32, [_vp, _i64, _i64, _i32, _vp, _vp]),
    'vtc_lambda_max_workspace_bytes': (_sz, [_i64]),
    'vtc_lambda_max': (_i32, [_vp, _i64, _vp, _vp, _sz, _vp]),
    'vtc_lambda_max_mirrored': (_i32, [_vp, _i64, _vp, _vp, _vp, _sz, _vp]),
    'vtc_fc_ista_fista_workspace_bytes': (_sz, [_i64, _i64, _i64, _i32]),
    'vtc_fc_ista_fista': (_i32, [_vp, _vp, _vp, _vp, _i64, _i64, _i64, _f32,
                                 _f32, _i32, _i32, _i32, _f32, _i32, _vp, _sz,
                                 ctypes.POINTER(_i32), _vp]),
    'vtc_fc_ista_fista_dev': (_i32, [_vp, _vp, _vp, _vp, _i64, _i64, _i64, _vp,
                                     _f32, _i32, _i32, _i32, _f32, _i32, _vp,
                                     _sz, ctypes.POINTER(_i32), _vp]),
    'vtc_group_gather_rows': (_i32, [_vp, _vp, _vp, _vp, _i64, _i64, _vp]),
    'vtc_group_gather_cols': (_i32, [_vp, _vp, _vp, _vp, _i64, _i64, _i64,
                                     _vp]),
    'vtc_group_scatter_add': (_i32, [_vp, _vp, _vp, _vp, _i64, _i64, _i64,
                                     _vp]),
    'vtc_subspace_ista_fista_workspace_bytes': (_sz, [_i64, _i64, _i64, _i64]),
    'vtc_subspace_ista_fista': (_i32, [_vp, _vp, _vp, _vp, _i64, _i64, _i64,
                                       _i64, _f32, _f32, _i32, _i32, _f32,
                                       _i32, _vp, _sz, ctypes.POINTER(_i32),
                                       _vp]),
    'vtc_conv_code_dims': (_i32, [_GEOM_P, ctypes.POINTER(ctypes.c_int32),
                                  ctypes.POINTER(ctypes.c_int32)]),
    'vtc_conv_ista_fista_workspace_bytes': (_sz, [_GEOM_P]),
    'vtc_conv_x3_supported': (_i32, [_GEOM_P]),
    'vtc_fc_residual': (_i32, [_vp, _vp, _vp, _vp, _i64, _i64, _i64, _vp]),
    'vtc_conv_residual': (_i32, [_vp, _vp, _vp, _vp, _GEOM_P, _vp]),
    'vtc_row_stats': (_i32, [_vp, _i64, _i64, _vp, _vp, _vp, _vp]),
    'vtc_group_norm_sum': (_i32, [_vp, _vp, _vp, _vp, _i64, _i64, _i64, _i64,
                                  _vp]),
    'vtc_window_minmax_workspace_bytes': (_sz, []),
    'vtc_window_minmax': (_i32, [_vp, _i64, _i64, _i64, _i64, _i64, _vp, _vp,
                                 _sz, _vp]),
    'vtc_rows_mean_abs_diff': (_i32, [_vp, _vp, _i64, _i64, _vp, _vp]),
    'vtc_whiten_center_surround_workspace_bytes': (_sz, [_i64, _i32, _i32,
                                                         _i32]),
    'vtc_whiten_center_surround': (_i32, [_vp, _vp, _i64, _i32, _i32, _i32,
                                          _f32, _f32, _i32, _vp, _sz, _vp]),
    'vtc_extract_patches': (_i32, [_vp, _vp, _vp, _vp, _vp, _i64, _i32, _i32,
                                   _i32, _i32, _i32, _vp]),
    'vtc_standardize_data_range': (_i32, [_vp, _vp, _i64, _vp, _vp, _sz, _vp]),
    'vtc_draw_patch_positions': (_i32, [_vp, _vp, _i64, _i32, _i32, _vp, _vp,
                                        _vp, _vp, _vp]),
    'vtc_ica_moment_workspace_bytes': (_sz, [_i64, _i64]),
    'vtc_ica_moment': (_i32, [_vp, _vp, _i64, _i64, _vp, _sz, _vp]),
    'vtc_ica_apply_workspace_bytes': (_sz, [_i64, _i64]),
    'vtc_ica_apply': (_i32, [_vp, _vp, _i64, _i64, _i64, _f32, _vp, _sz,
                             _vp]),
    'vtc_conv_ista_fista': (_i32, [_vp, _vp, _vp, _vp, _GEOM_P, _f32, _f32,
                                   _i32, _i32, _i32, _f32, _i32, _vp, _sz,
                                   ctypes.POINTER(_i32), _vp]),
    'vtc_fc_dict_gradient_workspace_bytes': (_sz, [_i64, _i64, _i64]),
    'vtc_fc_dict_gradient': (_i32, [_vp, _vp, _vp, _vp, _i64, _i64, _i64, _vp,
                                    _sz, _vp]),
    'vtc_subspace_alignment_gradient_workspace_bytes': (_sz, [_i64, _i64]),
    'vtc_subspace_alignment_gradient': (_i32, [_vp, _vp, _vp, _vp, _vp, _vp,
                                               _i64, _i64, _i64, _i64, _i32,
                                               _vp, _sz, _vp]),
    'vtc_fc_dict_apply': (_i32, [_vp, _vp, _vp, _vp, _f32, _i64, _f32, _f32,
                                 _i32, _i64, _i64, _vp]),
    'vtc_conv_dict_gradient_workspace_bytes': (_sz, [_GEOM_P]),
    'vtc_conv_dict_gradient': (_i32, [_vp, _vp, _vp, _vp, _GEOM_P, _i32, _vp,
                                      _sz, _vp]),
    'vtc_conv_dict_apply': (_i32, [_vp, _vp, _vp, _i64, _f32, _f32, _i32, _i64,
                                   _i64, _vp, _vp]),
    'vtc_code_energy_workspace_bytes': (_sz, [_i64, _i64, _i64]),
    'vtc_code_energy': (_i32, [_vp, _i64, _i64, _i64, _vp, _vp, _sz, _vp]),
    'vtc_hessian_ema': (_i32, [_vp, _vp, _i64, _i64, _vp]),
    'vtc_column_covariance_workspace_bytes': (_sz, [_i64, _i64]),
    'vtc_column_covariance': (_i32, [_vp, _i64, _i64, _i32, _vp, _vp, _vp,
                                     _vp, _sz, _vp]),
    'vtc_sym_eig_workspace_bytes': (_sz, [_i64]),
    'vtc_sym_eig': (_i32, [_vp, _i64, _i32, _vp, _vp, _vp, _vp, _sz, _vp]),
    'vtc_zca_matrices': (_i32, [_vp, _vp, _i64, ctypes.c_double, _vp, _vp,
                                _vp]),
    'vtc_row_transform': (_i32, [_vp, _i64, _i64, _vp, _vp, _f32, _vp, _vp]),
    'vtc_mat_inverse_workspace_bytes': (_sz, [_i64]),
    'vtc_mat_inverse': (_i32, [_vp, _i64, _vp, _vp, _vp, _sz, _vp]),
    'vtc_local_normalize_workspace_bytes': (_sz, [_i64, _i32, _i32, _i32,
                                                   ctypes.c_double]),
    'vtc_local_normalize': (_i32, [_vp, _vp, _vp, _i64, _i32, _i32, _i32,
                                   ctypes.c_double, _i32, _vp, _sz, _vp]),
    'vtc_column_moments_workspace_bytes': (_sz, [_i64, _i64]),
    'vtc_column_moments': (_i32, [_vp, _i32, _i64, _i64, _vp, _vp, _vp, _sz,
                                  _vp]),
    'vtc_column_apply': (_i32, [_vp, _i32, _i64, _i64, _i32, _vp, _vp, _vp]),
    'vtc_row_center': (_i32, [_vp, _i32, _i64, _i64, _vp, _vp, _vp]),
}

IMAGE_ABI_VERSION = 1

IMAGE_SIGNATURES = {
    'vtc_image_abi_version': (_i32, []),
    'vtc_img_filter_fd_workspace_bytes': (_sz, [_i64, _i32, _i32, _i32, _i32,
                                                _i32]),
    'vtc_img_filter_fd': (_i32, [_vp, _i32, _vp, _vp, _i64, _i32, _i32, _i32,
                                 _i32, _i32, _vp, _sz, _vp]),
    'vtc_img_filter_sd_workspace_bytes': (_sz, [_i64, _i32, _i32, _i32, _i32,
                                                _i32, _i32]),
    'vtc_img_filter_sd': (_i32, [_vp, _i32, _vp, _vp, _vp, _vp, _i64, _i32,
                                 _i32, _i32, _i32, _i32, _vp, _sz, _vp]),
    'vtc_img_tile_patches': (_i32, [_vp, _i32, _vp, _i64, _i32, _i32, _i32,
                                    _i32, _i32, _vp]),
    'vtc_img_assemble_patches': (_i32, [_vp, _i32, _vp, _vp, _i64, _i32, _i32,
                                        _i32, _i32, _i32, _i32, _vp]),
    'vtc_img_downsample': (_i32, [_vp, _i32, _vp, _i64, _i32, _i32, _i32,
                                  _i32, _vp]),
}

CODEC_ABI_VERSION = 1

CODEC_SIGNATURES = {
    'vtc_codec_abi_version': (_i32, []),
    'vtc_jpeg_quantize': (_i32, [_vp, _vp, _vp, _vp, _i64, _i32, _vp]),
    'vtc_jpeg_dequantize': (_i32, [_vp, _vp, _vp, _vp, _i64, _i32, _vp]),
    'vtc_jpeg_symbol_counts': (_i32, [_vp, _i64, _i32, _vp, _vp, _vp, _vp]),
    'vtc_jpeg_stream_bits': (_i32, [_vp, _i64, _i32, _vp, _vp, _vp, _vp,
                                    _vp]),
    'vtc_jpeg_bit_offsets_workspace_bytes': (_sz, [_i64]),
    'vtc_jpeg_bit_offsets': (_i32, [_vp, _i64, _vp, _vp, _sz, _vp]),
    'vtc_jpeg_pack': (_i32, [_vp, _i64, _i32, _vp, _vp, _vp, _vp, _vp, _vp,
                             _sz, _vp, _vp]),
}

DECODE_ABI_VERSION = 1

DECODE_SIGNATURES = {
    'vtc_decode_abi_version': (_i32, []),
    'vtc_jpeg_unpack_workspace_bytes': (_sz, []),
    'vtc_jpeg_unpack': (_i32, [_vp, _sz, _vp, _i64, _i32, _vp, _vp, _vp, _vp,
                               _vp, _vp, _vp, _sz, _vp]),
}

QUALITY_ABI_VERSION = 1

QUALITY_SIGNATURES = {
    'vtc_quality_abi_version': (_i32, []),
    'vtc_ssim_workspace_bytes': (_sz, [_i64, _i32, _i32]),
    'vtc_ssim': (_i32, [_vp, _vp, _i32, _vp, _vp, _vp, _i64, _i32, _i32, _vp,
                        _sz, _vp]),
}

STATS_ABI_VERSION = 1
STATS_MAX_IGNORE, STATS_MAX_BINS, STATS_MAX_JOINT_BINS = 8, 4096, 256

STATS_SIGNATURES = {
    'vtc_stats_abi_version': (_i32, []),
    'vtc_code_summary_workspace_bytes': (_sz, [_i64, _i64]),
    'vtc_code_summary': (_i32, [_vp, _i64, _i64, _vp, _i32, _vp, _vp, _vp,
                                _vp, _vp, _vp, _vp, _sz, _vp]),
    'vtc_code_histogram_workspace_bytes': (_sz, [_i64, _i64, _i32]),
    'vtc_code_histogram': (_i32, [_vp, _i64, _i64, _vp, _i32, _vp, _vp, _i32,
                                  _vp, _vp, _sz, _vp]),
    'vtc_code_joint_histogram_workspace_bytes': (_sz, [_i64, _i64]),
    'vtc_code_joint_histogram': (_i32, [_vp, _i64, _i64, _vp, _i64, _i32,
                                        _vp, _i32, _i32, _vp, _vp, _vp, _vp,
                                        _vp, _sz, _vp]),
    'vtc_binned_mean_workspace_bytes': (_sz, [_i64, _i32, _i32, _i32]),
    'vtc_binned_mean': (_i32, [_vp, _i32, _vp, _i64, _i32, _i32, _i32, _vp,
                               _vp, _vp, _sz, _vp]),
}

QUANT_ABI_VERSION = 1
QUANT_MAX_CODEWORDS, QUANT_ROWS = 1024, 512


class QuantState(ctypes.Structure):
  _fields_ = [('codebooks', ctypes.c_void_p), ('lengths', ctypes.c_void_p),
              ('counts', ctypes.c_void_p), ('cost', ctypes.c_void_p),
              ('k', ctypes.c_void_p), ('zero_index', ctypes.c_void_p),
              ('active', ctypes.c_void_p), ('iterations', ctypes.c_void_p)]


_QSTATE_P = ctypes.POINTER(QuantState)
_f64 = ctypes.c_double

QUANT_SIGNATURES = {
    'vtc_quant_abi_version': (_i32, []),
    'vtc_quant_assign': (_i32, [_vp, _i64, _i64, _vp, _vp, _vp, _i32, _f64,
                                _vp, _vp, _vp, _vp]),
    'vtc_quant_lloyd_step_workspace_bytes': (_sz, [_i64, _i64, _i32]),
    'vtc_quant_lloyd_step': (_i32, [_vp, _i64, _i64, _i32, _f64, _f64, _i32,
                                    _QSTATE_P, _QSTATE_P, _vp, _vp, _sz,
                                    _vp]),
    'vtc_quant_index_counts': (_i32, [_vp, _i64, _i64, _i32, _vp, _vp]),
}

VQ_ABI_VERSION = 1
VQ_MAX_DIM, VQ_MAX_CODEWORDS = 32, 4096
VQ_TILE_DOUBLES, VQ_ROWS = 4096, 2048


class VqState(ctypes.Structure):
  _fields_ = [('codebook', ctypes.c_void_p), ('lengths', ctypes.c_void_p),
              ('counts', ctypes.c_void_p), ('cost', ctypes.c_void_p),
              ('k', ctypes.c_void_p), ('zero_index', ctypes.c_void_p),
              ('active', ctypes.c_void_p), ('iterations', ctypes.c_void_p)]


_VQSTATE_P = ctypes.POINTER(VqState)

VQ_SIGNATURES = {
    'vtc_vq_abi_version': (_i32, []),
    'vtc_vq_assign': (_i32, [_vp, _i64, _i32, _vp, _vp, _vp, _i32, _f64, _vp,
                             _vp, _vp, _vp]),
    'vtc_vq_lloyd_step_workspace_bytes': (_sz, [_i64, _i32, _i32]),
    'vtc_vq_lloyd_step': (_i32, [_vp, _i64, _i32, _i32, _f64, _f64, _i32,
                                 _VQSTATE_P, _VQSTATE_P, _vp, _vp, _sz, _vp]),
    'vtc_vq_index_counts': (_i32, [_vp, _i64, _i32, _vp, _vp]),
}

INDEX_CODE_ABI_VERSION = 1
INDEX_CODE_ABSENT = 255
INDEX_CODE_MAX_COLUMNS, INDEX_CODE_MAX_SYMBOLS = 4096, 4096

INDEX_CODE_SIGNATURES = {
    'vtc_index_code_abi_version': (_i32, []),
    'vtc_index_code_bits': (_i32, [_vp, _i64, _i32, _vp, _i32, _vp, _vp, _vp,
                                   _vp]),
    'vtc_index_code_pack': (_i32, [_vp, _i64, _i32, _vp, _vp, _i32, _vp, _vp,
                                   _i64, _vp, _vp]),
}

INDEX_DECODE_ABI_VERSION = 1
INDEX_DECODE_LOOKUP_BITS = 10

INDEX_DECODE_SIGNATURES = {
    'vtc_index_decode_abi_version': (_i32, []),
    'vtc_index_code_unpack_workspace_bytes': (_sz, [_i32, _i32]),
    'vtc_index_code_unpack': (_i32, [_vp, _i64, _vp, _i64, _i32, _vp, _vp,
                                     _i32, _vp, _vp, _vp, _vp, _sz, _vp]),
}

INDEX_ANS_ABI_VERSION = 1
INDEX_ANS_PROB_BITS = 15
INDEX_ANS_LANES = 64
INDEX_ANS_MAX_STREAM_BITS = 24

INDEX_ANS_SIGNATURES = {
    'vtc_index_ans_abi_version': (_i32, []),
    'vtc_index_ans_workspace_bytes': (_sz, [_i32, _i32]),
    'vtc_index_ans_sizes': (_i32, [_vp, _i64, _i32, _vp, _i32, _i32, _vp, _vp,
                                   _vp, _sz, _vp]),
    'vtc_index_ans_pack': (_i32, [_vp, _i64, _i32, _vp, _i32, _i32, _vp, _vp,
                                  _vp, _i64, _vp, _vp, _sz, _vp]),
    'vtc_index_ans_unpack': (_i32, [_vp, _i64, _vp, _i64, _i32, _vp, _i32,
                                    _i32, _vp, _vp, _vp, _vp, _sz, _vp]),
}

VQ_LARGE_ABI_VERSION = 1
VQ_LARGE_MAX_CODEWORDS = 131072

VQ_LARGE_SIGNATURES = {
    'vtc_vq_large_abi_version': (_i32, []),
    'vtc_vq_large_assign': (_i32, [_vp, _i64, _i32, _vp, _vp, _vp, _i32, _f64,
                                   _vp, _vp, _vp, _vp]),
    'vtc_vq_large_lloyd_step_workspace_bytes': (_sz, [_i64, _i32, _i32]),
    'vtc_vq_large_lloyd_step': (_i32, [_vp, _i64, _i32, _i32, _f64, _f64,
                                       _i32, _VQSTATE_P, _VQSTATE_P, _vp, _vp,
                                       _sz, _vp]),
    'vtc_vq_large_index_counts': (_i32, [_vp, _i64, _i32, _vp, _vp]),
}


class VtcHipError(RuntimeError):
  pass


def load_library():
  global _lib
  if _lib is not None:
    return _lib
  if not LIBRARY_PATH.exists():
    raise ImportError(
        'libvtc_hip.so not found at %s -- build it with `make -C %s` '
        '(hipcc --offload-arch=gfx950).  There is no CPU fallback.'
        % (LIBRARY_PATH, _PKG_ROOT / 'csrc'))
  lib = ctypes.CDLL(str(LIBRARY_PATH), mode=os.RTLD_NOW)
  for table in (SIGNATURES, IMAGE_SIGNATURES, CODEC_SIGNATURES,
                DECODE_SIGNATURES, QUALITY_SIGNATURES, STATS_SIGNATURES,
                QUANT_SIGNATURES, VQ_SIGNATURES, INDEX_CODE_SIGNATURES,
                INDEX_DECODE_SIGNATURES, INDEX_ANS_SIGNATURES,
                VQ_LARGE_SIGNATURES):
    for name, (restype, argtypes) in table.items():
      fn = getattr(lib, name)
      fn.restype = restype
      fn.argtypes = argtypes
  if lib.vtc_abi_version() != ABI_VERSION:
    raise ImportError('libvtc_hip.so ABI version mismatch')
  if lib.vtc_image_abi_version() != IMAGE_ABI_VERSION:
    raise ImportError('libvtc_hip.so image ABI version mismatch')
  if lib.vtc_codec_abi_version() != CODEC_ABI_VERSION:
    raise ImportError('libvtc_hip.so codec ABI version mismatch')
  if lib.vtc_decode_abi_version() != DECODE_ABI_VERSION:
    raise ImportError('libvtc_hip.so decode ABI version mismatch')
  if lib.vtc_quality_abi_version() != QUALITY_ABI_VERSION:
    raise ImportError('libvtc_hip.so quality ABI version mismatch')
  if lib.vtc_stats_abi_version() != STATS_ABI_VERSION:
    raise ImportError('libvtc_hip.so stats ABI version mismatch')
  if lib.vtc_quant_abi_version() != QUANT_ABI_VERSION:
    raise ImportError('libvtc_hip.so quant ABI version mismatch')
  if lib.vtc_vq_abi_version() != VQ_ABI_VERSION:
    raise ImportError('libvtc_hip.so vector quantiser ABI version mismatch')
  if lib.vtc_index_code_abi_version() != INDEX_CODE_ABI_VERSION:
    raise ImportError('libvtc_hip.so index code ABI version mismatch')
  if lib.vtc_index_decode_abi_version() != INDEX_DECODE_ABI_VERSION:
    raise ImportError('libvtc_hip.so index decode ABI version mismatch')
  if lib.vtc_index_ans_abi_version() != INDEX_ANS_ABI_VERSION:
    raise ImportError('libvtc_hip.so index ANS ABI version mismatch')
  if lib.vtc_vq_large_abi_version() != VQ_LARGE_ABI_VERSION:
    raise ImportError('libvtc_hip.so large vector quantiser ABI version '
                      'mismatch')
  _lib = lib
  return lib


_prepared_devices = set()


def prepare_device(device):
  index = torch.device(device).index
  if index is None:
    index = torch.cuda.current_device()
  if index in _prepared_devices:
    return
  with torch.cuda.device(index):
    check(load_library().vtc_init(), 'vtc_init')
  _prepared_devices.add(index)


def check(status, what):
  if status == OK:
    return
  msg = load_library().vtc_last_error().decode('utf-8', 'replace')
  text = '%s: %s' % (what, msg)
  if status == ERR_UNSUPPORTED:
    raise NotImplementedError(text)
  if status == ERR_INVALID_ARGUMENT:
    raise ValueError(text)
  raise VtcHipError(text)


def require_device_tensor(t, name, dtype=torch.float32):
  if not torch.is_tensor(t):
    raise TypeError('%s must be a torch.Tensor' % name)
  if not t.is_cuda:
    raise VtcHipError(
        '%s lives on %s: the MI355X engine only runs on HIP device tensors '
        '(no CPU path is provided on purpose)' % (name, t.device))
  if t.dtype != dtype:
    raise TypeError('%s must be %s, got %s' % (name, dtype, t.dtype))
  return t


def aligned16(t):
  if t is None or t.data_ptr() % 16 == 0:
    return t
  return t.clone(memory_format=torch.contiguous_format)


def ptr(t):
  return ctypes.c_void_p(t.data_ptr()) if t is not None else ctypes.c_void_p(0)


def current_stream(device):
  return ctypes.c_void_p(torch.cuda.current_stream(device).cuda_stream)


def workspace(nbytes, device):
  return torch.empty(max(int(nbytes), 256), dtype=torch.uint8, device=device)


def threshold_mode(nonnegative_only, hard_threshold):
  if hard_threshold:
    return HARD_NONNEG if nonnegative_only else HARD
  return SOFT_NONNEG if nonnegative_only else SOFT


def variant_code(variant):
  assert variant in ['ista', 'fista']
  return FISTA if variant == 'fista' else ISTA


_default_precision = os.environ.get('VTC_PRECISION', 'auto')


def set_default_precision(name):
  global _default_precision
  assert name in ('auto',) + tuple(PRECISIONS)
  _default_precision = name


def get_default_precision():
  return _default_precision


kernel_timing = None


class timed_call(object):

  def __init__(self, device):
    self.device = device

  def __enter__(self):
    if kernel_timing is not None:
      self.start = torch.cuda.Event(enable_timing=True)
      self.stop = torch.cuda.Event(enable_timing=True)
      self.start.record(torch.cuda.current_stream(self.device))
    return self

  def __exit__(self, *exc):
    if kernel_timing is not None:
      self.stop.record(torch.cuda.current_stream(self.device))
      kernel_timing.append((self.start, self.stop))
    return False


def gram(matrix, transpose_a):
  lib = load_library()
  rows, cols = matrix.shape
  side = cols if transpose_a else rows
  out = torch.empty((side, side), dtype=torch.float32, device=matrix.device)
  check(lib.vtc_gram(ptr(matrix), rows, cols, 1 if transpose_a else 0,
                     ptr(out), current_stream(matrix.device)), 'vtc_gram')
  return out


LANCZOS_MAX_N = 1024
_use_device_eigensolver = os.environ.get('VTC_EIGEN', 'lanczos') != 'library'
spectrum_check = os.environ.get('VTC_SPECTRUM_CHECK', '1') != '0'
_pending_spectra = []


def _report_bad_spectrum(dictionary_for_message):
  print('the eigen-solve threw an exception. Likely due to one of the',
        'dictionary elements overflowing. The norm of each dictionary',
        'element is')
  flat = dictionary_for_message.reshape(dictionary_for_message.shape[0], -1)
  print(torch.norm(flat, dim=1, p=2))
  raise RuntimeError()


def poll_spectrum_checks(block=False):
  while _pending_spectra:
    event, pinned, dictionary = _pending_spectra[0]
    if block:
      event.synchronize()
    elif not event.query():
      return
    _pending_spectra.pop(0)
    lam = float(pinned[0])
    if not (lam == lam) or lam in (float('inf'), float('-inf')):
      del _pending_spectra[:]
      _report_bad_spectrum(dictionary)
    if float(pinned[2]) != 1.0:
      del _pending_spectra[:]
      _report_unconverged(lam)


def _report_unconverged(lam):
  raise RuntimeError(
      'the Lanczos eigen-solve had not converged at its step limit (top Ritz '
      'value %r still moving by more than 1e-6 per 8 steps)' % lam)


def lambda_max_device(gram_matrix, host_mirror=None):
  lib = load_library()
  n = gram_matrix.shape[0]
  out = torch.empty(3, dtype=torch.float32, device=gram_matrix.device)
  ws = workspace(lib.vtc_lambda_max_workspace_bytes(n), gram_matrix.device)
  check(lib.vtc_lambda_max_mirrored(
      ptr(gram_matrix), n, ptr(out),
      ctypes.c_void_p(host_mirror.data_ptr() if host_mirror is not None else 0),
      ptr(ws), ws.numel(), current_stream(gram_matrix.device)),
        'vtc_lambda_max')
  return out


def device_stepsize_available(n):
  return _use_device_eigensolver and n <= LANCZOS_MAX_N


def stepsize_on_device(gram_matrix, dictionary_for_message):
  poll_spectrum_checks()
  pinned = None
  if spectrum_check:
    pinned = torch.empty(3, dtype=torch.float32, pin_memory=True)
  out = lambda_max_device(gram_matrix, pinned)
  if spectrum_check:
    event = torch.cuda.Event()
    event.record(torch.cuda.current_stream(gram_matrix.device))
    _pending_spectra.append((event, pinned, dictionary_for_message))
  return out[1:2]


def stepsize_from_gram(gram_matrix, dictionary_for_message):
  n = gram_matrix.shape[0]
  unconverged = None
  try:
    if device_stepsize_available(n):
      out = lambda_max_device(gram_matrix)
      lipschitz_constant, stepsize, converged = [
          float(v) for v in out.tolist()]
      if not (lipschitz_constant == lipschitz_constant) or (
          lipschitz_constant in (float('inf'), float('-inf'))):
        raise RuntimeError('non-finite spectrum')
      if converged != 1.0:
        unconverged = lipschitz_constant
      else:
        return stepsize
    if unconverged is None:
      lipschitz_constant = torch.linalg.eigvalsh(gram_matrix, UPLO='U')[-1]
  except RuntimeError:
    _report_bad_spectrum(dictionary_for_message)
  if unconverged is not None:
    _report_unconverged(unconverged)
  return float(1. / lipschitz_constant)
```

Baseline: 1.695 million.

## Hand off final FISTA residual to dictionary gradient to skip recomputing it

On the last iteration the fused FISTA kernel now writes the residual (image minus reconstruction) to global memory, staging it through the LDS exchange area. The dictionary update reuses it for its first gradient step instead of recomputing E = X - A·D with a GEMM. Validity is tracked with tensor identity, version and an in-place-write epoch, and the momentum term is zeroed on the last iteration so the residual matches the final codes. The cost is an extra b×n write and more Python bookkeeping; correctness depends on the residual matching the codes after thresholding.

```diff
diff --git a/include/step/vtc_step.h b/include/step/vtc_step.h
--- /dev/null
+++ b/include/step/vtc_step.h
@@ -0,0 +1,41 @@
+#ifndef VTC_STEP_H_
+#define VTC_STEP_H_
+
+#include "../vtc_hip.h"
+
+#ifdef __cplusplus
+extern "C" {
+#endif
+
+#define VTC_STEP_ABI_VERSION 1
+
+int vtc_step_abi_version(void);
+
+int vtc_fc_ista_fista_residual_supported(int64_t b, int64_t n, int64_t s,
+                                         int precision, int threshold,
+                                         float early_stopping_epsilon);
+
+size_t vtc_fc_ista_fista_residual_workspace_bytes(int64_t b, int64_t n,
+                                                  int64_t s, int precision);
+
+int vtc_fc_ista_fista_residual(
+    const float* images, const float* dictionary, const float* initial_codes,
+    float* codes, int64_t b, int64_t n, int64_t s, float stepsize,
+    const float* stepsize_dev, float sparsity_weight, int num_iters,
+    int variant, int threshold, float early_stopping_epsilon, int precision,
+    void* workspace, size_t workspace_bytes, int* iters_run, void* stream,
+    float* residual);
+
+size_t vtc_fc_dict_gradient_from_residual_workspace_bytes(int64_t b, int64_t n,
+                                                          int64_t s);
+
+int vtc_fc_dict_gradient_from_residual(const float* codes,
+                                       const float* residual, float* grad_sum,
+                                       int64_t b, int64_t n, int64_t s,
+                                       void* workspace, size_t workspace_bytes,
+                                       void* stream);
+
+#ifdef __cplusplus
+}
+#endif
+#endif
diff --git a/vision-transform-codes_amd/analysis_transforms/fully_connected/ista_fista.py b/vision-transform-codes_amd/analysis_transforms/fully_connected/ista_fista.py
--- a/vision-transform-codes_amd/analysis_transforms/fully_connected/ista_fista.py
+++ b/vision-transform-codes_amd/analysis_transforms/fully_connected/ista_fista.py
@@ -38,30 +38,51 @@
   ws = vtc_hip.workspace(ws_bytes, images.device)
   codes = torch.empty((b, s), dtype=torch.float32, device=images.device)
   iters_run = ctypes.c_int(0)
+  stream = vtc_hip.current_stream(images.device)
   common = (int(num_iters), vtc_hip.variant_code(variant), mode, eps, prec,
-            vtc_hip.ptr(ws), ws.numel(), ctypes.byref(iters_run),
-            vtc_hip.current_stream(images.device))
+            vtc_hip.ptr(ws), ws.numel(), ctypes.byref(iters_run), stream)
+  residual = None
+  if (vtc_hip.residual_handoff_enabled() and
+      int(num_iters) <= 16384 and
+      lib.vtc_fc_ista_fista_residual_supported(b, n, s, prec, mode, eps)):
+    residual = torch.empty((b, n), dtype=torch.float32, device=images.device)
   if (stepsize is None and early_stopping_epsilon is None and
       vtc_hip.device_stepsize_available(n)):
     eta_dev = vtc_hip.stepsize_on_device(
         vtc_hip.gram(dictionary, transpose_a=True), dictionary)
     with vtc_hip.timed_call(images.device):
-      status = lib.vtc_fc_ista_fista_dev(
-          vtc_hip.ptr(images), vtc_hip.ptr(dictionary),
-          vtc_hip.ptr(initial_codes), vtc_hip.ptr(codes), b, n, s,
-          vtc_hip.ptr(eta_dev), lam, *common)
+      if residual is not None:
+        status = lib.vtc_fc_ista_fista_residual(
+            vtc_hip.ptr(images), vtc_hip.ptr(dictionary),
+            vtc_hip.ptr(initial_codes), vtc_hip.ptr(codes), b, n, s, 0.0,
+            vtc_hip.ptr(eta_dev), lam, *common, vtc_hip.ptr(residual))
+      else:
+        status = lib.vtc_fc_ista_fista_dev(
+            vtc_hip.ptr(images), vtc_hip.ptr(dictionary),
+            vtc_hip.ptr(initial_codes), vtc_hip.ptr(codes), b, n, s,
+            vtc_hip.ptr(eta_dev), lam, *common)
     vtc_hip.check(status, 'vtc_fc_ista_fista_dev')
   else:
     if stepsize is None:
       stepsize = vtc_hip.stepsize_from_gram(
           vtc_hip.gram(dictionary, transpose_a=True), dictionary)
     with vtc_hip.timed_call(images.device):
-      status = lib.vtc_fc_ista_fista(
-          vtc_hip.ptr(images), vtc_hip.ptr(dictionary),
-          vtc_hip.ptr(initial_codes), vtc_hip.ptr(codes), b, n, s,
-          float(stepsize), lam, *common)
+      if residual is not None:
+        status = lib.vtc_fc_ista_fista_residual(
+            vtc_hip.ptr(images), vtc_hip.ptr(dictionary),
+            vtc_hip.ptr(initial_codes), vtc_hip.ptr(codes), b, n, s,
+            float(stepsize), None, lam, *common, vtc_hip.ptr(residual))
+      else:
+        status = lib.vtc_fc_ista_fista(
+            vtc_hip.ptr(images), vtc_hip.ptr(dictionary),
+            vtc_hip.ptr(initial_codes), vtc_hip.ptr(codes), b, n, s,
+            float(stepsize), lam, *common)
     vtc_hip.check(status, 'vtc_fc_ista_fista')
   run.last_iters = iters_run.value
+  if residual is not None:
+    vtc_hip.handoff_stats['offered'] += 1
+    codes._vtc_handoff = vtc_hip.ResidualHandoff(
+        residual, images, dictionary, codes, images.device, stream.value)
   return codes
 
 
diff --git a/vision-transform-codes_amd/csrc/dict_update.hip b/vision-transform-codes_amd/csrc/dict_update.hip
--- a/vision-transform-codes_amd/csrc/dict_update.hip
+++ b/vision-transform-codes_amd/csrc/dict_update.hip
@@ -1,5 +1,6 @@
 #include "common.h"
 #include "gemm_f32.h"
+#include "../../include/step/vtc_step.h"
 
 namespace vtc {
 
@@ -245,6 +246,29 @@
   }
 };
 
+struct FcGradFromResidualLayout {
+  float* slabs;
+  FcGradFromResidualLayout(Carver& ws, int64_t b, int64_t n, int64_t s) {
+    slabs = ws.take<float>((size_t)gradient_slices(b, n, s) * s * n);
+  }
+};
+
+static int fc_gradient_from_residual(const float* codes, const float* E,
+                                     float* slabs, float* grad_sum, int64_t b,
+                                     int64_t n, int64_t s, hipStream_t st) {
+  if (b <= 512 && gemm_prefers_small(s, n)) {
+    EpiStore direct{grad_sum, n};
+    return launch_gemm_f32<false, false>(codes, s, E, n, s, n, b, 1, direct,
+                                         st);
+  }
+  const int slices = gradient_slices(b, n, s);
+  EpiSlab e2{slabs, s * n, n};
+  int rc = launch_gemm_f32<false, false>(codes, s, E, n, s, n, b, slices, e2,
+                                         st);
+  if (rc != VTC_OK) return rc;
+  return launch_slab_reduce(slabs, slices, s * n, grad_sum, st);
+}
+
 struct SlotGradLayout {
   float* slot_grad;
   SlotGradLayout(Carver& ws, int64_t slots, int64_t n) {
@@ -321,20 +345,37 @@
   hipStream_t st = as_stream(stream);
   Carver ws(workspace);
   const FcGradLayout L(ws, b, n, s);
-  const int slices = gradient_slices(b, n, s);
   EpiMinus e1{L.E, images, n, n};
   int rc = launch_gemm_f32<true, false>(codes, s, dictionary, n, b, n, s, 1,
                                         e1, st);
   if (rc != VTC_OK) return rc;
-  if (b <= 512 && gemm_prefers_small(s, n)) {
-    EpiStore direct{grad_sum, n};
-    return launch_gemm_f32<false, false>(codes, s, L.E, n, s, n, b, 1, direct,
-                                         st);
-  }
-  EpiSlab e2{L.slabs, s * n, n};
-  rc = launch_gemm_f32<false, false>(codes, s, L.E, n, s, n, b, slices, e2, st);
-  if (rc != VTC_OK) return rc;
-  return launch_slab_reduce(L.slabs, slices, s * n, grad_sum, st);
+  return fc_gradient_from_residual(codes, L.E, L.slabs, grad_sum, b, n, s, st);
+}
+
+extern "C" size_t vtc_fc_dict_gradient_from_residual_workspace_bytes(
+    int64_t b, int64_t n, int64_t s) {
+  if (b <= 0 || n <= 0 || s <= 0) return 256;
+  return measured_bytes<FcGradFromResidualLayout>(b, n, s);
+}
+
+extern "C" int vtc_fc_dict_gradient_from_residual(
+    const float* codes, const float* residual, float* grad_sum, int64_t b,
+    int64_t n, int64_t s, void* workspace, size_t workspace_bytes,
+    void* stream) {
+  VTC_REQUIRE(codes && residual && grad_sum,
+              "vtc_fc_dict_gradient_from_residual: null pointer");
+  VTC_REQUIRE(b > 0 && n > 0 && s > 0,
+              "vtc_fc_dict_gradient_from_residual: bad sizes");
+  if (!workspace ||
+      workspace_bytes <
+          vtc_fc_dict_gradient_from_residual_workspace_bytes(b, n, s)) {
+    set_error("vtc_fc_dict_gradient_from_residual: workspace too small");
+    return VTC_ERR_WORKSPACE;
+  }
+  Carver ws(workspace);
+  const FcGradFromResidualLayout L(ws, b, n, s);
+  return fc_gradient_from_residual(codes, residual, L.slabs, grad_sum, b, n, s,
+                                   as_stream(stream));
 }
 
 __global__ void sign_kernel(const float* __restrict__ x, float* __restrict__ y,
diff --git a/vision-transform-codes_amd/csrc/fc_fused.h b/vision-transform-codes_amd/csrc/fc_fused.h
--- a/vision-transform-codes_amd/csrc/fc_fused.h
+++ b/vision-transform-codes_amd/csrc/fc_fused.h
@@ -11,7 +11,8 @@
               int64_t s, float eta, const float* eta_dev,
               float sparsity_weight, int num_iters, int variant,
               int threshold, int precision, void* workspace,
-              size_t workspace_bytes, int* iters_run, hipStream_t st);
+              size_t workspace_bytes, int* iters_run, hipStream_t st,
+              float* residual = nullptr);
 int fused_max_iters();
 const float* fista_beta_table_on_this_device();
 
diff --git a/vision-transform-codes_amd/csrc/fc_fused.hip b/vision-transform-codes_amd/csrc/fc_fused.hip
--- a/vision-transform-codes_amd/csrc/fc_fused.hip
+++ b/vision-transform-codes_amd/csrc/fc_fused.hip
@@ -22,6 +22,7 @@
   const float* eta_dev;
   float lam;
   const float* dscale;
+  float* residual;
   unsigned long long* stamps;
 };
 
@@ -29,6 +30,7 @@
 constexpr int kRxRow = 528;
 constexpr int kYxPart = 32 * kYxRow;
 constexpr int kRxPart = 32 * kRxRow;
+constexpr int kResRow = 1040;
 
 template <int NPH, int NP>
 struct FusedLds {
@@ -40,9 +42,12 @@
   static constexpr int rx_bytes = NP * kRxPart;
   static constexpr int stat_bytes = 2 * 4 * 32 * 4;
   static constexpr int total = cst_bytes + yx_bytes + rx_bytes + stat_bytes;
+  static_assert(32 * kResRow <= (NP == 2 ? rx_bytes : yx_bytes + rx_bytes),
+                "the staged residual tile must fit the exchange area");
 };
 
-template <int NPH, int NP, int MODE, bool F16 = false, bool STAMP = false>
+template <int NPH, int NP, int MODE, bool F16 = false, bool STAMP = false,
+          bool RES = false>
 __global__ __launch_bounds__(256, 1) void fused_fista_kernel(FusedParams P) {
   static_assert(!F16 || NP == 2, "the f16 split exists as three products only");
   using L = FusedLds<NPH, NP>;
@@ -268,7 +273,7 @@
   };
   auto nothing = [](int) {};
 
-  auto exchange_r = [&]() {
+  auto exchange_r = [&](bool write_residual) {
     float v[2][16];
 #pragma unroll
     for (int nb = 0; nb < 2; ++nb)
@@ -324,17 +329,41 @@
         inv_sigma_y *= 1.f / f;
       }
     }
-#pragma unroll
-    for (int nb = 0; nb < 2; ++nb) {
-#pragma unroll
-      for (int g = 0; g < 4; ++g) {
-        const float v4[4] = {v[nb][4 * g], v[nb][4 * g + 1], v[nb][4 * g + 2],
-                             v[nb][4 * g + 3]};
-        uint2 hi, lo;
-        split_packed<F16, 4, NP == 2>(v4, hi, lo);
-        char* dst = Rx + rx_wr + 64 * nb + 16 * g;
-        *reinterpret_cast<uint2*>(dst) = hi;
-        if (NP == 2) *reinterpret_cast<uint2*>(dst + kRxPart) = lo;
+    if (RES && write_residual) {
+      char* stage = (NP == 2) ? Rx : Yx;
+      if (NP == 1) __syncthreads();
+      const float back = F16 ? 0.5f * inv_sigma_y : 1.f;
+#pragma unroll
+      for (int nb = 0; nb < 2; ++nb)
+#pragma unroll
+        for (int g = 0; g < 4; ++g)
+          *reinterpret_cast<float4*>(stage + r * kResRow +
+                                     4 * (64 * w + 32 * nb + 8 * g + 4 * h)) =
+              make_float4(v[nb][4 * g] * back, v[nb][4 * g + 1] * back,
+                          v[nb][4 * g + 2] * back, v[nb][4 * g + 3] * back);
+      __syncthreads();
+#pragma unroll
+      for (int j = 0; j < 8; ++j) {
+        const int row = 8 * w + j;
+        const int64_t out_patch = (int64_t)blockIdx.x * kFP + row;
+        if (out_patch < P.b)
+          *reinterpret_cast<float4*>(P.residual + out_patch * kFN + 4 * lane) =
+              *reinterpret_cast<const float4*>(stage + row * kResRow +
+                                               16 * lane);
+      }
+    } else {
+#pragma unroll
+      for (int nb = 0; nb < 2; ++nb) {
+#pragma unroll
+        for (int g = 0; g < 4; ++g) {
+          const float v4[4] = {v[nb][4 * g], v[nb][4 * g + 1],
+                               v[nb][4 * g + 2], v[nb][4 * g + 3]};
+          uint2 hi, lo;
+          split_packed<F16, 4, NP == 2>(v4, hi, lo);
+          char* dst = Rx + rx_wr + 64 * nb + 16 * g;
+          *reinterpret_cast<uint2*>(dst) = hi;
+          if (NP == 2) *reinterpret_cast<uint2*>(dst + kRxPart) = lo;
+        }
       }
     }
 #pragma unroll
@@ -352,7 +381,7 @@
       step3(p, p & 1, false, 0, nothing);
     }
   }
-  exchange_r();
+  exchange_r(false);
 
 #pragma unroll
   for (int i = 0; i < RING; ++i)
@@ -463,7 +492,8 @@
   };
 
   for (int it = 0; it < P.num_iters; ++it) {
-    const float beta = fista ? P.betas[it] : 0.f;
+    const bool last_out = RES && it == P.num_iters - 1;
+    const float beta = (fista && !last_out) ? P.betas[it] : 0.f;
     step1(0, 0, false, beta);
     VTC_STAMP(0)
 #pragma unroll
@@ -484,7 +514,7 @@
       }
       VTC_STAMP(3)
     }
-    exchange_r();
+    exchange_r(last_out);
     VTC_STAMP(4)
   }
   if (STAMP && lane == 0) {
@@ -527,7 +557,8 @@
 #undef VTC_SEG_PHASE
 }
 
-template <int NPH, int NP, int MODE, bool F16 = false, bool STAMP = false>
+template <int NPH, int NP, int MODE, bool F16 = false, bool STAMP = false,
+          bool RES = false>
 __global__ __launch_bounds__(256, 1) void fused_fista_kernel16(FusedParams P) {
   static_assert(!F16 || NP == 2, "the f16 split exists as three products only");
   using L = FusedLds<NPH, NP>;
@@ -785,7 +816,7 @@
   };
   auto nothing = [](int) {};
 
-  auto exchange_r = [&]() {
+  auto exchange_r = [&](bool write_residual) {
     float v[4][2][4];
 #pragma unroll
     for (int nb = 0; nb < 4; ++nb)
@@ -852,16 +883,42 @@
         }
       }
     }
-#pragma unroll
-    for (int nb = 0; nb < 4; ++nb) {
+    if (RES && write_residual) {
+      char* stage = (NP == 2) ? Rx : Yx;
+      if (NP == 1) __syncthreads();
 #pragma unroll
       for (int n = 0; n < 2; ++n) {
-        const float v4[4] = {v[nb][n][0], v[nb][n][1], v[nb][n][2], v[nb][n][3]};
-        uint2 hi, lo;
-        split_packed<F16, 4, NP == 2>(v4, hi, lo);
-        char* dst = Rx + rx_wr + 32 * nb + kRxHalf * n;
-        *reinterpret_cast<uint2*>(dst) = hi;
-        if (NP == 2) *reinterpret_cast<uint2*>(dst + kRxPart) = lo;
+        const float back = F16 ? 0.5f * inv_sigma_y[n] : 1.f;
+#pragma unroll
+        for (int nb = 0; nb < 4; ++nb)
+          *reinterpret_cast<float4*>(stage + (16 * n + c) * kResRow +
+                                     4 * (64 * w + 16 * nb + 4 * q)) =
+              make_float4(v[nb][n][0] * back, v[nb][n][1] * back,
+                          v[nb][n][2] * back, v[nb][n][3] * back);
+      }
+      __syncthreads();
+#pragma unroll
+      for (int j = 0; j < 8; ++j) {
+        const int row = 8 * w + j;
+        const int64_t out_patch = (int64_t)blockIdx.x * kFP + row;
+        if (out_patch < P.b)
+          *reinterpret_cast<float4*>(P.residual + out_patch * kFN + 4 * lane) =
+              *reinterpret_cast<const float4*>(stage + row * kResRow +
+                                               16 * lane);
+      }
+    } else {
+#pragma unroll
+      for (int nb = 0; nb < 4; ++nb) {
+#pragma unroll
+        for (int n = 0; n < 2; ++n) {
+          const float v4[4] = {v[nb][n][0], v[nb][n][1], v[nb][n][2],
+                               v[nb][n][3]};
+          uint2 hi, lo;
+          split_packed<F16, 4, NP == 2>(v4, hi, lo);
+          char* dst = Rx + rx_wr + 32 * nb + kRxHalf * n;
+          *reinterpret_cast<uint2*>(dst) = hi;
+          if (NP == 2) *reinterpret_cast<uint2*>(dst + kRxPart) = lo;
+        }
       }
     }
 #pragma unroll
@@ -882,7 +939,7 @@
       step3(p, p & 1, false, 0, nothing);
     }
   }
-  exchange_r();
+  exchange_r(false);
 
 #pragma unroll
   for (int i = 0; i < RING; ++i)
@@ -995,7 +1052,8 @@
   };
 
   for (int it = 0; it < P.num_iters; ++it) {
-    const float beta = fista ? P.betas[it] : 0.f;
+    const bool last_out = RES && it == P.num_iters - 1;
+    const float beta = (fista && !last_out) ? P.betas[it] : 0.f;
     step1(0, 0, false, beta);
     VTC_STAMP(0)
 #pragma unroll
@@ -1016,7 +1074,7 @@
       }
       VTC_STAMP(3)
     }
-    exchange_r();
+    exchange_r(last_out);
     VTC_STAMP(4)
   }
   if (STAMP && lane == 0) {
@@ -1104,18 +1162,19 @@
   return default_tile16(precision);
 }
 
-template <int NPH, int NP, int MODE, bool F16, bool STAMP, bool TILE16>
+template <int NPH, int NP, int MODE, bool F16, bool STAMP, bool TILE16,
+          bool RES = false>
 static auto fused_kernel() {
   if constexpr (TILE16)
-    return fused_fista_kernel16<NPH, NP, MODE, F16, STAMP>;
+    return fused_fista_kernel16<NPH, NP, MODE, F16, STAMP, RES>;
   else
-    return fused_fista_kernel<NPH, NP, MODE, F16, STAMP>;
-}
-
-template <int NPH, int NP, int MODE, bool F16, bool TILE16>
-static int launch_fused(const FusedParams& P, hipStream_t st) {
+    return fused_fista_kernel<NPH, NP, MODE, F16, STAMP, RES>;
+}
+
+template <int NPH, int NP, int MODE, bool F16, bool TILE16, bool RES>
+static int launch_fused_variant(const FusedParams& P, hipStream_t st) {
   using L = FusedLds<NPH, NP>;
-  auto kernel = fused_kernel<NPH, NP, MODE, F16, false, TILE16>();
+  auto kernel = fused_kernel<NPH, NP, MODE, F16, false, TILE16, RES>();
   static unsigned long long configured = 0;
   if (first_use_on_this_device(&configured)) {
     VTC_HIP_CHECK(hipFuncSetAttribute(
@@ -1126,6 +1185,13 @@
   hipLaunchKernelGGL(kernel, dim3(grid), dim3(256), L::total, st, P);
   VTC_LAUNCH_CHECK();
   return VTC_OK;
+}
+
+template <int NPH, int NP, int MODE, bool F16, bool TILE16>
+static int launch_fused(const FusedParams& P, hipStream_t st) {
+  return P.residual
+             ? launch_fused_variant<NPH, NP, MODE, F16, TILE16, true>(P, st)
+             : launch_fused_variant<NPH, NP, MODE, F16, TILE16, false>(P, st);
 }
 
 template <int NPH, int NP, bool F16, bool TILE16>
@@ -1164,7 +1230,7 @@
 template <int NPH, int NP, bool F16, bool TILE16>
 static int dispatch_mode(const FusedParams& P, int threshold, hipStream_t st) {
   static const bool stamps = getenv("VTC_FUSED_STAMPS") != nullptr;
-  if (stamps && threshold == VTC_SOFT && NPH == 8 && NP == 2)
+  if (stamps && !P.residual && threshold == VTC_SOFT && NPH == 8 && NP == 2)
     return launch_stamped<NPH, NP, F16, TILE16>(P, st);
   switch (threshold) {
     case VTC_SOFT: return launch_fused<NPH, NP, VTC_SOFT, F16, TILE16>(P, st);
@@ -1216,7 +1282,8 @@
               int64_t s, float eta, const float* eta_dev,
               float sparsity_weight, int num_iters, int variant,
               int threshold, int precision, void* workspace,
-              size_t workspace_bytes, int* iters_run, hipStream_t st) {
+              size_t workspace_bytes, int* iters_run, hipStream_t st,
+              float* residual) {
   if (!fused_shape_supported(b, n, s, precision)) {
     set_error("fused FISTA: unsupported shape");
     return VTC_ERR_UNSUPPORTED;
@@ -1273,6 +1340,7 @@
   P.lam = sparsity_weight;
   P.cutoff = sparsity_weight * eta;
   P.dscale = dscale;
+  P.residual = residual;
   P.stamps = nullptr;
   int rc;
   if (tile16)
diff --git a/vision-transform-codes_amd/csrc/fc_inference.hip b/vision-transform-codes_amd/csrc/fc_inference.hip
--- a/vision-transform-codes_amd/csrc/fc_inference.hip
+++ b/vision-transform-codes_amd/csrc/fc_inference.hip
@@ -5,6 +5,7 @@
 #include "fc_fused.h"
 #include "fused_stream.h"
 #include "fc_small.h"
+#include "../../include/step/vtc_step.h"
 
 #include <math.h>
 #include <vector>
@@ -267,7 +268,8 @@
                               int variant, int threshold,
                               float early_stopping_epsilon, int precision,
                               void* workspace, size_t workspace_bytes,
-                              int* iters_run, void* stream) {
+                              int* iters_run, void* stream,
+                              float* residual = nullptr) {
   VTC_REQUIRE(b >= 0 && n > 0 && s > 0, "vtc_fc_ista_fista: bad sizes");
   VTC_REQUIRE(b == 0 || (images && dictionary && codes),
               "vtc_fc_ista_fista: null pointer");
@@ -286,6 +288,36 @@
   const bool fused_ok = early_stopping_epsilon < 0.f &&
                         num_iters <= fused_max_iters() &&
                         fused_shape_supported(b, n, s, precision);
+  if (residual) {
+    if (!vtc_fc_ista_fista_residual_supported(b, n, s, precision, threshold,
+                                              early_stopping_epsilon) ||
+        num_iters > fused_max_iters()) {
+      set_error("vtc_fc_ista_fista_residual: only where the fused f16x3 kernel "
+                "runs (n == 256, s in {256, 512, 1024}, VTC_F16X3, no early "
+                "stopping, at most %d iterations)", fused_max_iters());
+      return VTC_ERR_UNSUPPORTED;
+    }
+    const char* odd = first_unaligned16({{"images", images},
+                                         {"dictionary", dictionary},
+                                         {"initial_codes", initial_codes},
+                                         {"codes", codes},
+                                         {"residual", residual}});
+    if (odd[0]) {
+      set_error("vtc_fc_ista_fista_residual: the fused kernel needs %s "
+                "16-byte aligned", odd);
+      return VTC_ERR_UNSUPPORTED;
+    }
+    if (!workspace || workspace_bytes <
+                          vtc_fc_ista_fista_residual_workspace_bytes(
+                              b, n, s, precision)) {
+      set_error("vtc_fc_ista_fista_residual: workspace too small");
+      return VTC_ERR_WORKSPACE;
+    }
+    return run_fused(images, dictionary, initial_codes, codes, b, n, s,
+                     stepsize, stepsize_dev, sparsity_weight, num_iters,
+                     variant, threshold, precision, workspace, workspace_bytes,
+                     iters_run, st, residual);
+  }
   if (precision == VTC_BF16 && !fused_ok) {
     set_error("vtc_fc_ista_fista: VTC_BF16 exists only as the fused kernel "
               "(n == 256, s in {256, 512, 1024}, no early stopping); use "
@@ -366,3 +398,42 @@
                             precision, workspace, workspace_bytes, iters_run,
                             stream);
 }
+
+extern "C" int vtc_step_abi_version(void) { return VTC_STEP_ABI_VERSION; }
+
+extern "C" int vtc_fc_ista_fista_residual_supported(
+    int64_t b, int64_t n, int64_t s, int precision, int threshold,
+    float early_stopping_epsilon) {
+  return precision == VTC_F16X3 && threshold >= VTC_SOFT &&
+                 threshold <= VTC_HARD_NONNEG &&
+                 early_stopping_epsilon < 0.f &&
+                 fused_shape_supported(b, n, s, precision)
+             ? 1
+             : 0;
+}
+
+extern "C" size_t vtc_fc_ista_fista_residual_workspace_bytes(int64_t b,
+                                                             int64_t n,
+                                                             int64_t s,
+                                                             int precision) {
+  if (precision != VTC_F16X3) return 256;
+  return fused_workspace_bytes(b, n, s, precision);
+}
+
+extern "C" int vtc_fc_ista_fista_residual(
+    const float* images, const float* dictionary, const float* initial_codes,
+    float* codes, int64_t b, int64_t n, int64_t s, float stepsize,
+    const float* stepsize_dev, float sparsity_weight, int num_iters,
+    int variant, int threshold, float early_stopping_epsilon, int precision,
+    void* workspace, size_t workspace_bytes, int* iters_run, void* stream,
+    float* residual) {
+  VTC_REQUIRE(b > 0 && n > 0 && s > 0,
+              "vtc_fc_ista_fista_residual: bad sizes");
+  VTC_REQUIRE(images && dictionary && codes && residual,
+              "vtc_fc_ista_fista_residual: null pointer");
+  return fc_ista_fista_impl(images, dictionary, initial_codes, codes, b, n, s,
+                            stepsize, stepsize_dev, sparsity_weight, num_iters,
+                            variant, threshold, early_stopping_epsilon,
+                            precision, workspace, workspace_bytes, iters_run,
+                            stream, residual);
+}
diff --git a/vision-transform-codes_amd/dict_update_rules/convolutional/_common.py b/vision-transform-codes_amd/dict_update_rules/convolutional/_common.py
--- a/vision-transform-codes_amd/dict_update_rules/convolutional/_common.py
+++ b/vision-transform-codes_amd/dict_update_rules/convolutional/_common.py
@@ -50,3 +50,4 @@
         vtc_hip.ptr(hessian_diagonal), total_batch, float(stepsize),
         float(lowest_code_val), 1 if normalize_dictionary else 0, s,
         kernel_elems, vtc_hip.ptr(scratch), stream), 'vtc_conv_dict_apply')
+    vtc_hip.note_inplace_write()
diff --git a/vision-transform-codes_amd/dict_update_rules/fully_connected/_common.py b/vision-transform-codes_amd/dict_update_rules/fully_connected/_common.py
--- a/vision-transform-codes_amd/dict_update_rules/fully_connected/_common.py
+++ b/vision-transform-codes_amd/dict_update_rules/fully_connected/_common.py
@@ -8,6 +8,10 @@
             normalize_dictionary, hessian_diagonal=None, lowest_code_val=0.001,
             penalty=None):
   lib = vtc_hip.load_library()
+  handoff = getattr(codes, '_vtc_handoff', None) if torch.is_tensor(
+      codes) else None
+  if handoff is not None:
+    del codes._vtc_handoff
   images = vtc_hip.require_device_tensor(images, 'images').contiguous()
   codes = vtc_hip.require_device_tensor(codes, 'codes').contiguous()
   vtc_hip.require_device_tensor(dictionary, 'dictionary')
@@ -25,11 +29,23 @@
                          device)
   grad_sum = parallel.take((s, n), device)
   total_batch = parallel.global_batch(b, device)
-  for _ in range(num_iters):
-    vtc_hip.check(lib.vtc_fc_dict_gradient(
-        vtc_hip.ptr(images), vtc_hip.ptr(dictionary), vtc_hip.ptr(codes),
-        vtc_hip.ptr(grad_sum), b, n, s, vtc_hip.ptr(ws), ws.numel(), stream),
-        'vtc_fc_dict_gradient')
+  if handoff is not None and not (
+      vtc_hip.residual_handoff_enabled() and num_iters > 0 and
+      handoff.matches(images, dictionary, codes, device, stream.value)):
+    handoff = None
+  for it in range(num_iters):
+    if it == 0 and handoff is not None:
+      vtc_hip.check(lib.vtc_fc_dict_gradient_from_residual(
+          vtc_hip.ptr(codes), vtc_hip.ptr(handoff.residual),
+          vtc_hip.ptr(grad_sum), b, n, s, vtc_hip.ptr(ws), ws.numel(),
+          stream), 'vtc_fc_dict_gradient_from_residual')
+      vtc_hip.handoff_stats['taken'] += 1
+      handoff = None
+    else:
+      vtc_hip.check(lib.vtc_fc_dict_gradient(
+          vtc_hip.ptr(images), vtc_hip.ptr(dictionary), vtc_hip.ptr(codes),
+          vtc_hip.ptr(grad_sum), b, n, s, vtc_hip.ptr(ws), ws.numel(),
+          stream), 'vtc_fc_dict_gradient')
     parallel.all_reduce_sum_(grad_sum)
     pen_weight, pen_grad = 0.0, None
     if penalty is not None:
@@ -41,3 +57,4 @@
         float(pen_weight), total_batch, float(stepsize),
         float(lowest_code_val), 1 if normalize_dictionary else 0, s, n,
         stream), 'vtc_fc_dict_apply')
+    vtc_hip.note_inplace_write()
diff --git a/vision-transform-codes_amd/dict_update_rules/fully_connected/ica_natural_gradient.py b/vision-transform-codes_amd/dict_update_rules/fully_connected/ica_natural_gradient.py
--- a/vision-transform-codes_amd/dict_update_rules/fully_connected/ica_natural_gradient.py
+++ b/vision-transform-codes_amd/dict_update_rules/fully_connected/ica_natural_gradient.py
@@ -27,3 +27,4 @@
         vtc_hip.ptr(dictionary), vtc_hip.ptr(moment), total, s, n,
         float(stepsize), vtc_hip.ptr(ws), ws.numel(), stream),
         'vtc_ica_apply')
+    vtc_hip.note_inplace_write()
diff --git a/vision-transform-codes_amd/vtc_hip/__init__.py b/vision-transform-codes_amd/vtc_hip/__init__.py
--- a/vision-transform-codes_amd/vtc_hip/__init__.py
+++ b/vision-transform-codes_amd/vtc_hip/__init__.py
@@ -310,7 +310,6 @@
     'vtc_vq_large_index_counts': (_i32, [_vp, _i64, _i32, _vp, _vp]),
 }
 
-
 class VtcHipError(RuntimeError):
   pass
 
@@ -324,12 +323,13 @@
         'libvtc_hip.so not found at %s -- build it with `make -C %s` '
         '(hipcc --offload-arch=gfx950).  There is no CPU fallback.'
         % (LIBRARY_PATH, _PKG_ROOT / 'csrc'))
+  from vtc_hip import step as _step
   lib = ctypes.CDLL(str(LIBRARY_PATH), mode=os.RTLD_NOW)
   for table in (SIGNATURES, IMAGE_SIGNATURES, CODEC_SIGNATURES,
                 DECODE_SIGNATURES, QUALITY_SIGNATURES, STATS_SIGNATURES,
                 QUANT_SIGNATURES, VQ_SIGNATURES, INDEX_CODE_SIGNATURES,
                 INDEX_DECODE_SIGNATURES, INDEX_ANS_SIGNATURES,
-                VQ_LARGE_SIGNATURES):
+                VQ_LARGE_SIGNATURES, _step.STEP_SIGNATURES):
     for name, (restype, argtypes) in table.items():
       fn = getattr(lib, name)
       fn.restype = restype
@@ -359,6 +359,8 @@
   if lib.vtc_vq_large_abi_version() != VQ_LARGE_ABI_VERSION:
     raise ImportError('libvtc_hip.so large vector quantiser ABI version '
                       'mismatch')
+  if lib.vtc_step_abi_version() != _step.STEP_ABI_VERSION:
+    raise ImportError('libvtc_hip.so step ABI version mismatch')
   _lib = lib
   return lib
 
@@ -463,6 +465,49 @@
       self.stop.record(torch.cuda.current_stream(self.device))
       kernel_timing.append((self.start, self.stop))
     return False
+
+
+_residual_handoff = os.environ.get('VTC_RESIDUAL_HANDOFF', '1') != '0'
+handoff_stats = {'offered': 0, 'taken': 0}
+
+inplace_epoch = 0
+
+
+def set_residual_handoff(enabled):
+  global _residual_handoff
+  _residual_handoff = bool(enabled)
+
+
+def residual_handoff_enabled():
+  return _residual_handoff
+
+
+def note_inplace_write():
+  global inplace_epoch
+  inplace_epoch += 1
+
+
+def tensor_identity(t):
+  return (t.data_ptr(), tuple(t.shape), t._version)
+
+
+class ResidualHandoff(object):
+
+  def __init__(self, residual, images, dictionary, codes, device, stream):
+    self.residual = residual
+    self.images = tensor_identity(images)
+    self.dictionary = tensor_identity(dictionary)
+    self.codes = tensor_identity(codes)
+    self.device = device
+    self.stream = stream
+    self.epoch = inplace_epoch
+
+  def matches(self, images, dictionary, codes, device, stream):
+    return (self.epoch == inplace_epoch and self.device == device and
+            self.stream == stream and
+            self.images == tensor_identity(images) and
+            self.dictionary == tensor_identity(dictionary) and
+            self.codes == tensor_identity(codes))
 
 
 def gram(matrix, transpose_a):
diff --git a/vision-transform-codes_amd/vtc_hip/step.py b/vision-transform-codes_amd/vtc_hip/step.py
--- /dev/null
+++ b/vision-transform-codes_amd/vtc_hip/step.py
@@ -0,0 +1,25 @@
+import ctypes
+
+_i64 = ctypes.c_int64
+_i32 = ctypes.c_int
+_f32 = ctypes.c_float
+_vp = ctypes.c_void_p
+_sz = ctypes.c_size_t
+
+STEP_ABI_VERSION = 1
+
+STEP_SIGNATURES = {
+    'vtc_step_abi_version': (_i32, []),
+    'vtc_fc_ista_fista_residual_supported': (_i32, [_i64, _i64, _i64, _i32,
+                                                    _i32, _f32]),
+    'vtc_fc_ista_fista_residual_workspace_bytes': (_sz, [_i64, _i64, _i64,
+                                                         _i32]),
+    'vtc_fc_ista_fista_residual': (_i32, [_vp, _vp, _vp, _vp, _i64, _i64,
+                                          _i64, _f32, _vp, _f32, _i32, _i32,
+                                          _i32, _f32, _i32, _vp, _sz, _vp,
+                                          _vp, _vp]),
+    'vtc_fc_dict_gradient_from_residual_workspace_bytes': (_sz, [_i64, _i64,
+                                                                 _i64]),
+    'vtc_fc_dict_gradient_from_residual': (_i32, [_vp, _vp, _vp, _i64, _i64,
+                                                  _i64, _vp, _sz, _vp]),
+}
```

Result: no change. 1.704 million (median of 6 runs) (+0.5%).
